# bdwsq1996/Effi-MVS-plus

Hardware: AMD Instinct MI355X
Metric: ref-views/sec (cost-volume hot path: warp + cost volume + 3-D regularisation + cascaded GRU refinement) (higher is better)
Workload: dtype f32 (3x3 MFMA convs: products as 3 bf16 partial products hi*hi+hi*lo+lo*hi, f32 accumulate; all else f32); 1 GPU; cfg3: DTU-shaped 1600x1184, N=5 views (S=4 sources), 3-stage cascade ndepths=48,8,8, GRU iters 3,3,3, seeded-random weights, features of the stock FPN resident in HBM; parallelism=single GPU, views_in_flight=3, arithmetic=split

## Files before the change

effi_mvs_plus_amd/_lib.py:

```python
from __future__ import annotations

import ctypes as C
import os
import threading

_HERE = os.path.dirname(os.path.abspath(__file__))
LIB_PATH = os.environ.get("EFFI_MVS_LIB") or os.path.join(_HERE, "libeffimvs_hip.so")
HEADER_PATH = os.path.join(os.path.dirname(_HERE), "include", "effi_mvs_hip.h")

_vp, _i, _l, _f, _d = C.c_void_p, C.c_int, C.c_long, C.c_float, C.c_double

SIGNATURES = {
    "effi_version": [],
    "effi_set_workspace": [_i, _vp, _l],
    "effi_set_option": [C.c_char_p, _l],
    "effi_launch_form": [_i, _i, _i, _i, _i, _i, _i, _i, _vp],
    "effi_fusion_dynamic_filter_f32": [_vp, _vp, _vp, _vp, _i, _i, _i, _vp, _i, _i, _f, _i, _f, _f, _i, _vp, _vp, _vp, _vp, _vp, _vp,
                                       _vp, _vp],
    "effi_fusion_dtu_filter_f32": [_vp, _vp, _vp, _vp, _i, _i, _i, _vp, _f, _f, _i, _i, _f, _f, _vp, _vp, _vp, _vp, _vp, _vp, _vp],
    "effi_fusion_dtu_filter_scan_f32": [_vp, _vp, _i, _vp, _vp, _i, _i, _i, _i, _vp, _f, _f, _i, _i, _f, _f, _vp, _vp, _vp, _vp, _vp, _vp, _vp],
    "effi_fusion_dynamic_filter_scan_f32": [_vp, _vp, _i, _vp, _vp, _i, _i, _i, _i, _vp, _i, _i, _f, _i, _f, _f, _i, _vp, _vp, _vp, _vp, _vp,
                                            _vp, _vp],
    "effi_fusion_static_filter_f32": [_vp, _vp, _vp, _vp, _i, _i, _i, _vp, _i, _i, _f, _d, _d, _d, _vp, _vp, _vp, _vp, _vp, _vp, _vp, _vp,
                                      _vp],
# ... 10 lines not shown
    "effi_fusion_gipuma_view_f32": [_vp, _vp, _vp, _i, _i, _vp, _vp, _i, _i, _i, _f, _i, _f, _f, _vp, _vp, _vp, _vp, _vp, _vp, _vp],
    "effi_dtu_cell_keys_f32": [_vp, _l, _d, _i, _i, _i, _i, _i, _i, _vp, _vp],
    "effi_dtu_reduce_blocks": [_l],
    "effi_dtu_reduce_round_f32": [_vp, _vp, _l, _i, _i, _i, _d, _vp, _vp, _vp, _vp],
    "effi_dtu_nn_capped_f32": [_vp, _l, _vp, _vp, _l, _d, _i, _i, _i, _i, _i, _i, _d, _vp, _vp],
    "effi_dtu_obs_mask_f32": [_vp, _l, _d, _d, _d, _d, _vp, _i, _i, _i, _vp, _vp],
    "effi_dtu_above_plane_f32": [_vp, _l, _d, _d, _d, _d, _vp, _vp],
    "effi_metrics_blocks": [_l],
    "effi_mvs_loss_f32": [_vp, _vp, _vp, _vp, _i, _i, _vp, _vp, _vp, _vp, _vp, _vp],
    "effi_mvs_loss_bwd_f32": [_vp, _vp, _vp, _vp, _i, _i, _vp, _vp, _vp, _vp, _vp],
    "effi_depth_metrics_f32": [_vp, _vp, _vp, _i, _l, _i, _vp, _i, _vp, _vp, _i, _vp, _vp, _vp, _vp, _vp, _vp],
    "effi_adamw_max_tensors": [],
    "effi_adamw_multi_f32": [_vp, _vp, _vp, _vp, _vp, _vp, _i, _d, _vp, _d, _d, _d, _d, _vp],
    "effi_gradnorm_max_tensors": [],
    "effi_gradnorm_chunks": [_vp, _i],
    "effi_gradnorm_partial_f32": [_vp, _vp, _i, _vp, _vp],
    "effi_gradnorm_finish_f32": [_vp, _l, _d, _vp, _vp, _vp],
    "effi_adamw_multi_clip_f32": [_vp, _vp, _vp, _vp, _vp, _vp, _i, _d, _vp, _d, _d, _d, _d, _vp, _i, _vp],
    "effi_fusion_vis_filter_f32": [_vp, _vp, _i, _i, _i, _i, _f, _f, _i, _i, _vp, _vp],
    "effi_fusion_points_f32": [_i, _vp, _l, _vp, _vp, _i, _i, _i, _vp, _vp, _vp],
    "effi_fusion_dtu_reproject_f32": [_vp, _vp, _vp, _vp, _i, _i, _i, _i, _f, _f, _vp, _vp, _vp, _vp],
    "effi_compose_rel_proj_f32": [_vp, _i, _vp, _vp],
    "effi_rel_proj_f32": [_vp, _vp, _vp, _vp],
    "effi_planar_to_nhwc_f32": [_vp, _vp, _i, _i, _i, _vp],
    "effi_homo_warp_f32": [_vp, _vp, _vp, _l, _l, _i, _i, _i, _i, _vp, _vp],
    "effi_warpcorr_views_f32": [_vp, _vp, _i, _vp, _vp, _l, _l, _i, _i, _i, _i, _vp, _vp, _vp],
    "effi_warpcorr_views_tbl_f32": [_vp, _i, _vp, _vp, _l, _l, _i, _i, _i, _i, _vp, _vp, _vp],
    "effi_warpcorr_views_x3_f32": [_vp, _vp, _i, _vp, _vp, _l, _l, _i, _i, _i, _i, _vp, _vp, _i, _vp],
    "effi_warpcorr_views_x3_tbl_f32": [_vp, _i, _vp, _vp, _l, _l, _i, _i, _i, _i, _vp, _vp, _i, _vp],
    "effi_warpcorr_dyn_tbl_f32": [_vp, _i, _vp, _vp, _vp, _vp, _i, _i, _i, _i, _i, _vp, _vp, _vp],
    "effi_view_table_set": [_vp, _vp, _i, _vp],
    "effi_pixelwise_net_f32": [_vp, _vp, _i, _i, _i, _vp, _vp],
    "effi_view_aggregate_f32": [_vp, _vp, _i, _i, _i, _vp, _vp],
    "effi_warpcorr_dyn_f32": [_vp, _vp, _i, _vp, _vp, _vp, _vp, _i, _i, _i, _i, _i, _vp, _vp, _vp],
    "effi_conv3d_k3_f32": [_vp, _vp, _i, _vp, _vp, _i, _i, _i, _i, _i, _i, _i, _vp, _vp, _vp],
    "effi_deconv3d_k3s2_bf16x3_f32": [_vp, _i, _vp, _vp, _i, _i, _i, _i, _i, _vp, _vp, _vp],
    "effi_conv3d_k3s2_mfma_f32": [_vp, _i, _vp, _vp, _i, _i, _i, _i, _i, _vp, _vp],
    "effi_conv3d_k3s1_mfma_f32": [_vp, _i, _vp, _vp, _i, _i, _i, _i, _i, _vp, _vp],
    "effi_deconv3d_k3_f32": [_vp, _i, _vp, _vp, _i, _i, _i, _i, _i, _i, _vp, _vp, _vp],
    "effi_softmax_regress_conf_f32": [_vp, _vp, _l, _l, _i, _i, _vp, _vp, _vp, _i, _vp, _vp],
    "effi_softmax_regress_conf_up_f32": [_vp, _vp, _l, _l, _i, _i, _i, _vp, _vp, _vp, _i, _vp, _vp, _i, _vp],
    "effi_vol_lookup1d_f32": [_vp, _l, _l, _i, _vp, _l, _l, _l, _i, _vp, _vp, _l, _i, _i, _vp, _vp],
    "effi_bilinear_sampler1d_f32": [_vp, _i, _i, _i, _vp, _l, _vp, _vp, _vp],
    "effi_getcost_conv1x1_f32": [_vp, _vp, _i, _i, _vp, _vp, _l, _l, _i, _vp, _l, _l, _i, _vp, _vp, _l, _i, _i, _i, _vp, _vp, _i,
                                 _i, _vp, _vp],
    "effi_getcost_f32": [_vp, _vp, _i, _i, _vp, _vp, _l, _l, _i, _vp, _l, _l, _i, _vp, _vp, _l, _i, _i, _i, _vp, _vp],
    "effi_conv2d_f32": [_vp, _vp, _i, _vp, _vp, _i, _i, _i, _i, _i, _i, _vp, _vp, _vp, _i, _vp, _vp, _vp],
    "effi_conv3d_k3s1_roll_bf16x3_f32": [_vp, _vp, _i, _vp, _vp, _i, _i, _i, _i, _i, _vp, _vp],
    "effi_conv3d_k3s1_bf16x3_f32": [_vp, _vp, _i, _vp, _vp, _i, _i, _i, _i, _i, _vp, _vp],
    "effi_vol_lookup1d_pair_f32": [_vp, _vp, _l, _l, _i, _vp, _l, _l, _l, _i, _vp, _vp, _l, _i, _i, _vp, _vp, _vp],
    "effi_conv3d_k3_pair_f32": [_vp, _vp, _vp, _vp, _vp, _vp, _vp, _vp, _i, _i, _i, _i, _i, _i, _i, _vp],
    "effi_conv3d_k3s1_roll_bf16x3_pair_f32": [_vp, _vp, _vp, _vp, _vp, _vp, _vp, _vp, _vp, _i, _i, _i, _i, _i, _i, _vp],
    "effi_csp_gen_roll_bf16x3_pair_f32": [_vp, _i, _i, _i] + [_vp] * 16 + [_vp],
    "effi_debug_poison_lds": [C.c_uint, _vp, _vp],
    "effi_debug_pk_war_probe": [_vp, _i, _i, _i, _vp],
    "effi_deconv3d_k3_pair_f32": [_vp, _vp, _vp, _vp, _vp, _vp, _vp, _vp, _i, _i, _i, _i, _i, _i, _i, _vp],
    "effi_homo_warp_bwd_f32": [_vp, _vp, _l, _l, _i, _i, _i, _i, _vp, _vp, _vp],
    "effi_warpcorr_views_bwd_f32": [_vp, _vp, _i, _vp, _vp, _l, _l, _i, _i, _i, _i, _vp, _vp, _vp, _vp],
    "effi_image_prepare_u8_f32": [_vp, _i, _i, _i, _i, _i, _vp, _vp],
    "effi_resize_linear_f32": [_vp, _i, _i, _i, _i, _i, _vp, _vp],
    "effi_images_prepare_batch_u8_f32": [_vp, _i, _i, _i, _vp, _vp],
    "effi_gt_pyramid_f32": [_vp, _vp, _i, _vp, _i, _i, _i, _vp, _vp, _vp],
    "effi_encoder_inputs_f32": [_vp, _vp, _i, _vp, _vp, _l, _l, _i, _vp, _l, _l, _i, _vp, _vp, _l, _i, _i, _i, _vp, _vp, _vp, _vp,
                                _i, _vp, _vp, _vp],
    "effi_encoder_inputs_bf16x3_f32": [_vp, _vp, _i, _vp, _vp, _l, _l, _i, _vp, _l, _l, _i, _vp, _vp, _l, _i, _i, _i, _vp, _vp, _vp, _vp,
                                       _i, _vp, _vp, _vp],
    "effi_conv2d_k3_bf16x3_pair_f32": [_vp, _vp, _i, _vp, _vp, _vp, _vp, _vp, _i, _vp, _vp, _vp, _i, _i, _i, _i, _vp],
    "effi_conv2d_k3_k1_up2x_bf16x3_f32": [_vp, _vp, _i, _vp, _vp, _i, _vp, _vp, _vp, _vp, _i, _i, _i, _vp, _vp, _vp],
    "effi_conv2d_k3_k1_bf16x3_f32": [_vp, _vp, _i, _vp, _vp, _i, _i, _vp, _i, _vp, _vp, _i, _i, _i, _i, _vp, _vp],
    "effi_conv2d_k3_bf16x3_f32": [_vp, _vp, _i, _vp, _vp, _i, _i, _i, _i, _i, _vp, _vp, _vp, _i, _vp, _vp, _vp],
    "effi_conv2d_k5s2_f32": [_vp, _i, _vp, _vp, _i, _i, _i, _i, _vp, _vp],
    "effi_conv2d_k5s2_bf16x3_f32": [_vp, _i, _vp, _vp, _i, _i, _i, _i, _vp, _vp],
    "effi_conv3d_k3s2_bf16x3_f32": [_vp, _i, _vp, _vp, _i, _i, _i, _i, _i, _vp, _vp],
    "effi_conv2d_c1k7_relu_f32": [_vp, _vp, _vp, _i, _i, _i, _vp, _vp],
    "effi_conv2d_c1k7_relu_bf16x3_f32": [_vp, _vp, _vp, _i, _i, _i, _vp, _vp],
    "effi_convex_upsample2x_f32": [_vp, _vp, _vp, _i, _i, _i, _vp, _vp, _vp, _vp],
    "effi_compose_rel_proj_stages_f32": [_vp, _i, _i, _vp, _vp],
    "effi_cascade_setup_f32": [_vp, _i, _i, _vp, _vp, _vp, _i, _i, _vp, _vp],
    "effi_split_tanh_relu_stages_f32": [_vp, _vp, _vp, _vp, _vp, _vp, _i, _vp],
    "effi_split_tanh_relu_f32": [_vp, _i, _i, _i, _vp, _vp, _vp],
    "effi_depth_to_inv_f32": [_vp, _vp, _i, _i, _vp, _vp],
    "effi_stage1_hypotheses_f32": [_vp, _i, _i, _vp, _vp, _vp],
    "effi_upsample_nearest_f32": [_vp, _i, _i, _i, _i, _vp, _vp],
    "effi_head_update_f32": [_vp, _vp, _vp, _vp, _i, _i, _i, _vp, _vp, _vp],
    "effi_conv2d_k3_twice_bf16x3_f32": [_vp, _i, _vp, _vp, _vp, _vp, _i, _i, _i, _vp, _vp],
    "effi_conv2d_f32_batch": [_vp, _vp, _i, _vp, _vp, _i, _i, _i, _i, _i, _i, _vp, _vp, _vp, _i, _vp, _vp, _i, _vp, _l, _l, _vp],
    "effi_conv2d_k3_bf16x3_f32_batch": [_vp, _vp, _i, _vp, _vp, _i, _i, _i, _i, _i, _vp, _vp, _vp, _i, _vp, _vp, _i, _vp, _l, _l, _vp],
    "effi_conv2d_k5s2_f32_batch": [_vp, _i, _vp, _vp, _i, _i, _i, _i, _vp, _i, _l, _l, _vp],
    "effi_conv2d_k5s2_bf16x3_f32_batch": [_vp, _i, _vp, _vp, _i, _i, _i, _i, _vp, _i, _l, _l, _vp],
    "effi_conv2d_k3_twice_bf16x3_f32_batch": [_vp, _i, _vp, _vp, _vp, _vp, _i, _i, _i, _vp, _i, _l, _l, _vp],
    "effi_compose_rel_proj_f32_batch": [_vp, _i, _vp, _i, _l, _l, _vp],
    "effi_cascade_setup_f32_batch": [_vp, _i, _i, _vp, _vp, _vp, _i, _i, _vp, _i, _l, _l, _l, _vp, _l, _vp],
    "effi_warpcorr_views_f32_batch": [_vp, _vp, _i, _vp, _vp, _l, _l, _i, _i, _i, _i, _vp, _vp, _i, _l, _l, _l, _l, _l, _l, _vp],
    "effi_warpcorr_views_x3_f32_batch": [_vp, _vp, _i, _vp, _vp, _l, _l, _i, _i, _i, _i, _vp, _vp, _i, _i, _l, _l, _l, _l, _l, _l, _vp],
    "effi_view_aggregate_f32_batch": [_vp, _vp, _i, _i, _i, _vp, _i, _l, _l, _l, _vp],
    "effi_softmax_regress_conf_f32_batch": [_vp, _vp, _l, _l, _i, _i, _vp, _vp, _vp, _i, _vp, _i, _l, _l, _l, _l, _l, _l, _vp],
    "effi_softmax_regress_conf_up_f32_batch": [_vp, _vp, _l, _l, _i, _i, _i, _vp, _vp, _vp, _i, _vp, _vp, _i, _i, _l, _l, _l, _l, _l, _l,
                                               _l, _vp],
    "effi_conv3d_k3_f32_batch": [_vp, _vp, _i, _vp, _vp, _i, _i, _i, _i, _i, _i, _i, _vp, _vp, _i, _vp, _l, _l, _vp],
    "effi_deconv3d_k3_f32_batch": [_vp, _i, _vp, _vp, _i, _i, _i, _i, _i, _i, _vp, _vp, _i, _l, _l, _l, _vp],
    "effi_conv3d_k3s1_mfma_f32_batch": [_vp, _i, _vp, _vp, _i, _i, _i, _i, _i, _vp, _i, _l, _l, _vp],
    "effi_conv3d_k3s2_mfma_f32_batch": [_vp, _i, _vp, _vp, _i, _i, _i, _i, _i, _vp, _i, _l, _l, _vp],
    "effi_conv3d_k3s1_bf16x3_f32_batch": [_vp, _vp, _i, _vp, _vp, _i, _i, _i, _i, _i, _vp, _i, _vp, _l, _vp],
    "effi_conv3d_k3s1_roll_bf16x3_f32_batch": [_vp, _vp, _i, _vp, _vp, _i, _i, _i, _i, _i, _vp, _i, _vp, _l, _vp],
    "effi_conv3d_k3s2_bf16x3_f32_batch": [_vp, _i, _vp, _vp, _i, _i, _i, _i, _i, _vp, _i, _l, _l, _vp],
    "effi_deconv3d_k3s2_bf16x3_f32_batch": [_vp, _i, _vp, _vp, _i, _i, _i, _i, _i, _vp, _vp, _i, _l, _l, _l, _vp],
# ... 106 lines not shown
```

effi_mvs_plus_amd/csrc/api.hip:

```cpp
#include "common.hpp"
#include "launch_form.hpp"
#include <cstdlib>
#include <cstring>
#include <mutex>

extern "C" int effi_version(void) { return 200; }

extern "C" const char* effi_error_string(int code) {
    switch (code) {
        case EFFI_OK: return "ok";
        case EFFI_ERR_BADARG: return "bad argument (null pointer, non-positive size, or inconsistent shapes)";
        case EFFI_ERR_UNSUPPORTED: return "shape / channel count not instantiated in this build";
        case EFFI_ERR_LAUNCH: return "kernel launch failed (hipPeekAtLastError)";
        case EFFI_ERR_WORKSPACE: return "no workspace registered for the current device (effi_set_workspace)";
        default: return "unknown error code";
    }
}

static const void* g_workspace[EFFI_MAX_DEVICES];

extern "C" long effi_workspace_bytes(void) { return 256; }

extern "C" int effi_set_workspace(int device, void* workspace, long bytes) {
    if (device < 0 || device >= EFFI_MAX_DEVICES) return EFFI_ERR_BADARG;
    if (workspace != nullptr && bytes < effi_workspace_bytes()) return EFFI_ERR_BADARG;
    __atomic_store_n(&g_workspace[device], (const void*)workspace, __ATOMIC_RELEASE);
    return EFFI_OK;
}

extern "C" const void* effi_get_workspace(int device) {
    if (device < 0 || device >= EFFI_MAX_DEVICES) return nullptr;
    return __atomic_load_n(&g_workspace[device], __ATOMIC_ACQUIRE);
}

const float* effi_zero_page() {
    int dev = -1;
    if (hipGetDevice(&dev) != hipSuccess) return nullptr;
    return (const float*)effi_get_workspace(dev);
}

namespace {
const char* const kOptName[EFFI_OPT_COUNT] = {"warp_lds_kb", "dyn_form", "dyn_setup_exact", "dyn_xchg", "pixnet_mfma", "force_mr", "mr4_min",
                                              "mr4_nt2_max", "mr2_min", "wide_tiles", "roll_mr", "roll_zt", "roll_rp", "deconv_mr", "sr_waves", "enc_gen_mr3", "c3_lean", "dyn_win",
                                              "roll_slide"};
long g_opt[EFFI_OPT_COUNT];
std::once_flag g_opt_once;
void load_options() {
    for (int i = 0; i < EFFI_OPT_COUNT; ++i) {
        char env[64] = "EFFI_";
        size_t n = strlen(env);
        for (const char* c = kOptName[i]; *c && n + 1 < sizeof(env); ++c) env[n++] = (*c >= 'a' && *c <= 'z') ? (char)(*c - 32) : *c;
        env[n] = 0;
        const char* v = getenv(env);
        g_opt[i] = (v && *v) ? atol(v) : EFFI_OPT_UNSET;
    }
}
int find_option(const char* name) {
    if (!name) return -1;
    for (int i = 0; i < EFFI_OPT_COUNT; ++i)
        if (strcmp(name, kOptName[i]) == 0) return i;
    return -1;
}
}

long effi_option(int id) {
    std::call_once(g_opt_once, load_options);
    return __atomic_load_n(&g_opt[id], __ATOMIC_RELAXED);
}

extern "C" int effi_set_option(const char* name, long value) {
    const int id = find_option(name);
    if (id < 0) return EFFI_ERR_BADARG;
    std::call_once(g_opt_once, load_options);
    __atomic_store_n(&g_opt[id], value, __ATOMIC_RELAXED);
    return EFFI_OK;
}

extern "C" long effi_get_option(const char* name) {
    const int id = find_option(name);
    return id < 0 ? EFFI_OPT_UNSET : effi_option(id);
}

extern "C" long effi_option_unset(void) { return EFFI_OPT_UNSET; }

extern "C" int effi_launch_form(int launcher, int nt, int h, int w, int planes, int count, int cout, int flags, int* form) {
    if (!form || nt < 1 || h < 1 || w < 1 || planes < 1 || count < 1 || cout < 1) return EFFI_ERR_BADARG;
    const bool sr = flags & EFFI_LF_FLAG_SR, zb = flags & EFFI_LF_FLAG_ZB, k1 = flags & EFFI_LF_FLAG_K1, s2 = flags & EFFI_LF_FLAG_S2;
    const EffiFormOpts o = effi_form_opts();
    EffiForm f;
    switch (launcher) {
        case EFFI_LF_X3: f = effi_pick_x3(nt, h, w, zb ? planes : 1, zb, sr, o); break;
        case EFFI_LF_X3_BATCH: f = effi_pick_x3_batch(nt, h, w, count, o); break;
        case EFFI_LF_X3_ZB_BATCH: f = effi_pick_x3_zb_batch(nt, h, w, (long)planes * count, o); break;
        case EFFI_LF_X3_PAIR: f = effi_pick_x3_pair(nt, h, w, sr, o); break;
        case EFFI_LF_CONV2D: f = effi_pick_generic(k1 ? 1 : 3, h, w, count); break;
        case EFFI_LF_PLANES3D: f = effi_pick_planes(h, w, (long)planes * count, s2 ? 2 : 4); break;
        case EFFI_LF_K5S2: f = effi_pick_planes(h, w, count, 2); break;
        case EFFI_LF_S2_X3: f = effi_pick_s2_x3(h, w, nt == 1 ? 1 : (nt + 1) / 2, (long)planes * count); break;
        case EFFI_LF_ROLL: f = effi_pick_roll((flags & EFFI_LF_FLAG_OCT2) ? 2 : 1, nt, cout, h, w, planes, count, o); break;
        case EFFI_LF_DECONV_X3: f = effi_pick_deconv_x3(cout, h, w, planes, count, o); break;
        case EFFI_LF_C3_PLANES: f = effi_pick_c3_planes(h, w, planes, count); break;
        case EFFI_LF_DECONV_K3: f = effi_pick_deconv_k3(cout, h, w, planes, count); break;
        case EFFI_LF_C3_ZPT: f = EffiForm{1, EFFI_C3_TX, 4, effi_pick_c3_zpt(s2 ? 2 : 1, s2 ? 2 : 1, h, w, planes, nt, count), 0}; break;
        default: return EFFI_ERR_BADARG;
    }
    form[0] = f.rows, form[1] = f.cols, form[2] = f.waves, form[3] = f.planes, form[4] = f.variant;
    return EFFI_OK;
}

namespace {
__global__ __launch_bounds__(256) void lds_poison_kernel(unsigned pattern, unsigned* sink) {
    __shared__ unsigned buf[16 * 1024];
    for (int i = threadIdx.x; i < 16 * 1024; i += 256) buf[i] = pattern;
    __syncthreads();
    if (buf[(threadIdx.x * 61) & 16383] != pattern) sink[0] = 1;
}
}

extern "C" int effi_debug_poison_lds(unsigned pattern, void* sink4, effi_stream_t stream) {
    if (!sink4) return EFFI_ERR_BADARG;
    hipLaunchKernelGGL(lds_poison_kernel, dim3(2048), dim3(256), 0, effi_s(stream), pattern, reinterpret_cast<unsigned*>(sink4));
    EFFI_LAUNCH_CHECK();
    return EFFI_OK;
}

namespace {
template <int VARIANT>
__global__ __launch_bounds__(256) void pk_war_probe_kernel(float* __restrict__ out, int reps) {
    const int tid = blockIdx.x * 256 + threadIdx.x;
    const float x = 1.0f + (float)(tid & 15) * 0.0625f, y = 2.0f, bad = 1000.0f, w = 1.0f;
    float r0, r1;
    asm volatile(
        "v_mov_b32 v10, %2\n"
        "v_mov_b32 v11, %3\n"
        "v_mov_b32 v12, 0\n"
        "v_mov_b32 v13, 0\n"
        "v_mov_b32 v14, %5\n"
        "v_mov_b32 v15, %5\n"
        "s_nop 7\n"
        "s_mov_b32 s20, %6\n"
        "1:\n"
        ".rept 16\n"
        ".if %c7 == 3\n"
        "v_fma_f32 v12, v10, v14, v12\n"
        "v_fma_f32 v13, v11, v14, v13\n"
        ".else\n"
        "v_pk_fma_f32 v[12:13], v[10:11], v[14:15], v[12:13] op_sel_hi:[1,0,1]\n"
        ".endif\n"
        ".if %c7 == 1\n"
        "s_nop 0\n"
        ".endif\n"
        ".if %c7 == 2\n"
        "v_pk_mov_b32 v[10:11], v[16:17], v[10:11] op_sel:[0,1]\n"
        ".else\n"
// ... 31 lines not shown
```

effi_mvs_plus_amd/csrc/common.hpp:

```cpp
#pragma once
#include <hip/hip_runtime.h>
#include "../../include/effi_mvs_hip.h"

#define EFFI_LAUNCH_CHECK()                                   \
    do {                                                      \
        if (hipPeekAtLastError() != hipSuccess) return EFFI_ERR_LAUNCH; \
    } while (0)

const float* effi_zero_page();

enum EffiOption {
    EFFI_OPT_WARP_LDS_KB,
    EFFI_OPT_DYN_FORM,
    EFFI_OPT_DYN_SETUP_EXACT,
    EFFI_OPT_DYN_XCHG,
    EFFI_OPT_PIXNET_MFMA,
    EFFI_OPT_FORCE_MR,
    EFFI_OPT_MR4_MIN, EFFI_OPT_MR4_NT2_MAX, EFFI_OPT_MR2_MIN,
    EFFI_OPT_WIDE_TILES,
    EFFI_OPT_ROLL_MR, EFFI_OPT_ROLL_ZT, EFFI_OPT_ROLL_RP,
    EFFI_OPT_DECONV_MR,
    EFFI_OPT_SR_WAVES,
    EFFI_OPT_ENC_GEN_MR3,
    EFFI_OPT_C3_LEAN,
    EFFI_OPT_DYN_WIN,
    EFFI_OPT_ROLL_SLIDE,
    EFFI_OPT_COUNT
};
constexpr long EFFI_OPT_UNSET = -0x7fffffffL;
long effi_option(int id);

static inline hipStream_t effi_s(effi_stream_t s) {
    (void)hipGetLastError();
    return reinterpret_cast<hipStream_t>(s);
}
static inline int effi_cdiv(long a, long b) { return (int)((a + b - 1) / b); }

struct EffiPtrList {
    const float* p[EFFI_MAX_VIEWS + 1];
    const float* const* tbl;
};
__device__ __forceinline__ const float* effi_resolve_views(const float* ref, const EffiPtrList& l) {
    return l.tbl ? l.tbl[0] : ref;
}
struct EffiOutList {
    float* p[EFFI_MAX_VIEWS + 1];
};

__device__ __forceinline__ float effi_dpp_f(float v, int ctrl_sel) {
    int i = __float_as_int(v);
    int r;
    switch (ctrl_sel) {
        case 0:  r = __builtin_amdgcn_update_dpp(0, i, 0xB1, 0xF, 0xF, true); break;
        case 1:  r = __builtin_amdgcn_update_dpp(0, i, 0x4E, 0xF, 0xF, true); break;
        default: r = __builtin_amdgcn_update_dpp(0, i, 0x141, 0xF, 0xF, true); break;
    }
    return __int_as_float(r);
}

template <int LPP>
__device__ __forceinline__ float effi_group_sum(float v) {
    static_assert(LPP == 1 || LPP == 2 || LPP == 4 || LPP == 8, "lanes per pixel");
    if (LPP >= 2) v += effi_dpp_f(v, 0);
    if (LPP >= 4) v += effi_dpp_f(v, 1);
    if (LPP >= 8) v += effi_dpp_f(v, 2);
    return v;
}
template <int LPP>
__device__ __forceinline__ float effi_group_max(float v) {
    if (LPP >= 2) v = fmaxf(v, effi_dpp_f(v, 0));
    if (LPP >= 4) v = fmaxf(v, effi_dpp_f(v, 1));
    if (LPP >= 8) v = fmaxf(v, effi_dpp_f(v, 2));
    return v;
}

__device__ __forceinline__ int effi_xcd_remap(int bid, int nblocks) {
    const int q = nblocks >> 3, r = nblocks & 7;
    const int xcd = bid & 7, idx = bid >> 3;
    const int base = (xcd < r) ? xcd * (q + 1) : r * (q + 1) + (xcd - r) * q;
// ... 54 lines not shown
        intervals[threadIdx.x] = base * ratio;
    } else if (threadIdx.x == 3) {
        intervals[3] = 1.0f / hi;
    } else if (threadIdx.x == 4) {
        intervals[4] = 1.0f / lo;
    }
}

__device__ __forceinline__ float effi_lk_rcp(float b) {
#ifdef EFFI_EXACT_LOOKUP
    return 1.0f / b;
#else
    const float r0 = __builtin_amdgcn_rcpf(b);
    return fmaf(fmaf(-b, r0, 1.0f), r0, r0);
#endif
}
__device__ __forceinline__ float effi_lk_div(float a, float b, float rb) {
#ifdef EFFI_EXACT_LOOKUP
    (void)rb;
    return a / b;
#else
    const float q = a * rb;
    return fmaf(fmaf(-q, b, a), rb, q);
#endif
}

__device__ __forceinline__ void lookup1d_index(int Dp, float q_depth, float dmin, float dmax, int& x0, float& w0, float& w1) {
    const float scaled = effi_lk_rcp(q_depth);
    const float min_disp = effi_lk_rcp(dmax), max_disp = effi_lk_rcp(dmin);
    const float den = (max_disp - min_disp) + 1e-10f;
    const float disp = effi_lk_div(scaled - min_disp, den, effi_lk_rcp(den));
    const float dm1 = (float)(Dp - 1);
    const float t = disp * dm1;
    const float g = effi_lk_div(2.0f * t, dm1, effi_lk_rcp(dm1)) - 1.0f;
    float ix = ((g + 1.0f) * 0.5f) * dm1;
    ix = fminf(fmaxf(ix, -2.0f), dm1 + 2.0f);
    const float x0f = floorf(ix);
    x0 = (int)x0f;
    w1 = ix - x0f;
    w0 = (x0f + 1.0f) - ix;
}
__device__ __forceinline__ int lookup1d_tap0(int Dp, int x0) { return min(max(x0, 0), Dp - 1); }
__device__ __forceinline__ int lookup1d_tap1(int Dp, int x0) { return min(max(x0 + 1, 0), Dp - 1); }
__device__ __forceinline__ float lookup1d_blend(int Dp, int x0, float w0, float w1, float v0, float v1) {
    const bool in0 = (x0 >= 0) & (x0 <= Dp - 1), in1 = (x0 + 1 >= 0) & (x0 + 1 <= Dp - 1);
    float r = in0 ? v0 * w0 : 0.0f;
    r = in1 ? r + v1 * w1 : r;
    return r;
}
__device__ __forceinline__ float lookup1d_fetch(const float* __restrict__ vol, long dstride, int Dp, int x0, float w0, float w1) {
    const float v0 = vol[lookup1d_tap0(Dp, x0) * dstride], v1 = vol[lookup1d_tap1(Dp, x0) * dstride];
    return lookup1d_blend(Dp, x0, w0, w1, v0, v1);
}
__host__ __device__ inline bool effi_vol_fits32(long npix, long ps, int D, long ds) {
    return ps >= 0 && ds >= 0 && npix >= 1 && D >= 1 && ((npix - 1) * ps + (long)(D - 1) * ds + 1) * 4 < (1L << 31);
}
__host__ __device__ inline bool effi_lookup_fits32(long npix, long cps, int Dcur, long cds, long rps, int Dreg, long rds) {
    return effi_vol_fits32(npix, cps, Dcur, cds) && effi_vol_fits32(npix, rps, Dreg, rds);
}
template <int NQ>
__device__ __forceinline__ void effi_getcost_pixel(float inv_or_depth, int input_is_depth, const float* __restrict__ disp_range, int n_range,
                                                   float itv, const float* __restrict__ cur_vol, long cpo, long cds, int Dcur,
                                                   const float* __restrict__ reg_vol, long rpo, long rds, int Dreg, float rlo, float rhi,
                                                   bool off32, float (&cost)[2 * NQ]) {
    float depth = inv_or_depth;
    if (!input_is_depth) depth = effi_inv_to_depth(depth, disp_range[0], disp_range[n_range - 1]);
    const float dv = effi_lk_rcp(depth);
    const float half = (float)(NQ / 2) * itv;
    const float smin = fmaxf(dv - half, 1e-4f);
    const float smax = fminf(fmaxf(dv + half, 1e-4f), 1e4f);
    const float step = (smax - smin) / (float)(NQ - 1);
    constexpr int QB = NQ <= 3 ? NQ : 2;
    static_assert(NQ % QB == 0, "whole batches");
#pragma unroll
    for (int k0 = 0; k0 < NQ; k0 += QB) {
        int xc[QB], xr[QB];
        float wc0[QB], wc1[QB], wr0[QB], wr1[QB];
#pragma unroll
        for (int k = 0; k < QB; ++k) {
            const float s = fmaxf(smin + (float)(k0 + k) * step, 1e-5f);
            const float qd = effi_lk_rcp(s);
            lookup1d_index(Dcur, qd, rlo, rhi, xc[k], wc0[k], wc1[k]);
            xr[k] = xc[k]; wr0[k] = wc0[k]; wr1[k] = wc1[k];
            if (Dreg != Dcur) lookup1d_index(Dreg, qd, rlo, rhi, xr[k], wr0[k], wr1[k]);
        }
        float vc0[QB], vc1[QB], vr0[QB], vr1[QB];
        if (off32) {
            const unsigned cb = (unsigned)cpo * 4u, rb = (unsigned)rpo * 4u, cs = (unsigned)cds * 4u, rs = (unsigned)rds * 4u;
            const char* cbase = reinterpret_cast<const char*>(cur_vol);
            const char* rbase = reinterpret_cast<const char*>(reg_vol);
#pragma unroll
            for (int k = 0; k < QB; ++k) {
                vc0[k] = *reinterpret_cast<const float*>(cbase + (size_t)(cb + (unsigned)lookup1d_tap0(Dcur, xc[k]) * cs));
                vc1[k] = *reinterpret_cast<const float*>(cbase + (size_t)(cb + (unsigned)lookup1d_tap1(Dcur, xc[k]) * cs));
                vr0[k] = *reinterpret_cast<const float*>(rbase + (size_t)(rb + (unsigned)lookup1d_tap0(Dreg, xr[k]) * rs));
                vr1[k] = *reinterpret_cast<const float*>(rbase + (size_t)(rb + (unsigned)lookup1d_tap1(Dreg, xr[k]) * rs));
            }
        } else {
            const float* __restrict__ cur = cur_vol + cpo;
            const float* __restrict__ reg = reg_vol + rpo;
#pragma unroll
            for (int k = 0; k < QB; ++k) {
                vc0[k] = cur[lookup1d_tap0(Dcur, xc[k]) * cds];
                vc1[k] = cur[lookup1d_tap1(Dcur, xc[k]) * cds];
                vr0[k] = reg[lookup1d_tap0(Dreg, xr[k]) * rds];
                vr1[k] = reg[lookup1d_tap1(Dreg, xr[k]) * rds];
// ... 192 lines not shown
```

effi_mvs_plus_amd/csrc/conv3d.hip:

```cpp
#include "common.hpp"
#include "launch_form.hpp"

namespace {

constexpr int TX = EFFI_C3_TX, TY = EFFI_C3_TY;
static_assert(TX * TY == 256, "one thread per tile pixel");

struct SrcSet {
    const float* p[EFFI_MAX_SRC];
    int ch[EFFI_MAX_SRC];
};

__device__ __forceinline__ const float* src_channel(const SrcSet& s, int c, long plane) {
    if (c < s.ch[0]) return s.p[0] + (long)c * plane;
    c -= s.ch[0];
    if (c < s.ch[1]) return s.p[1] + (long)c * plane;
    c -= s.ch[1];
    return s.p[2] + (long)c * plane;
}

template <int COUT_T, int SZ, int SXY, int ZPT, bool DENSE>
__device__ __forceinline__ void conv3d_k3_body(SrcSet src, int cin, const float* __restrict__ wgt,
                                               const float* __restrict__ bias, int cout,
                                               int D, int h, int w, int Do, int ho, int wo,
// ... 121 lines not shown

template <int COUT_T, int SZ, int SXY, int ZPT, bool DENSE = false>
__global__ __launch_bounds__(256) void conv3d_k3_kernel(SrcSet src, int cin, const float* __restrict__ wgt,
                                                        const float* __restrict__ bias, int cout,
                                                        int D, int h, int w, int Do, int ho, int wo,
                                                        int relu, const float* __restrict__ skip,
                                                        float* __restrict__ out) {
    conv3d_k3_body<COUT_T, SZ, SXY, ZPT, DENSE>(src, cin, wgt, bias, cout, D, h, w, Do, ho, wo, relu, skip, out);
}

struct C3Batch {
    long src[EFFI_MAX_SRC];
    long skip, out;
};
template <int COUT_T, int SZ, int SXY, int ZPT, bool DENSE = false>
__global__ __launch_bounds__(256) void conv3d_k3_batch_kernel(SrcSet src, C3Batch bt, int cin, const float* __restrict__ wgt,
                                                              const float* __restrict__ bias, int cout, int D, int h, int w, int Do,
                                                              int ho, int wo, int relu, const float* __restrict__ skip,
                                                              float* __restrict__ out) {
    const long smp = blockIdx.y;
#pragma unroll
    for (int i = 0; i < EFFI_MAX_SRC; ++i) src.p[i] += smp * bt.src[i];
    conv3d_k3_body<COUT_T, SZ, SXY, ZPT, DENSE>(src, cin, wgt, bias, cout, D, h, w, Do, ho, wo, relu, skip ? skip + smp * bt.skip : nullptr,
                                                out + smp * bt.out);
}

struct Conv3dCall {
    SrcSet src;
    const float* wgt;
    const float* bias;
    const float* skip;
    float* out;
};
template <int COUT_T, int SZ, int SXY, int ZPT>
__global__ __launch_bounds__(256) void conv3d_k3_pair_kernel(Conv3dCall a, Conv3dCall b, int cin, int cout, int D, int h, int w,
                                                             int Do, int ho, int wo, int relu) {
    const bool second = blockIdx.y != 0;
    SrcSet src;
#pragma unroll
    for (int i = 0; i < EFFI_MAX_SRC; ++i) {
        src.p[i] = second ? b.src.p[i] : a.src.p[i];
        src.ch[i] = second ? b.src.ch[i] : a.src.ch[i];
    }
    conv3d_k3_body<COUT_T, SZ, SXY, ZPT, true>(src, cin, second ? b.wgt : a.wgt, second ? b.bias : a.bias, cout, D, h, w, Do, ho, wo,
                                               relu, second ? b.skip : a.skip, second ? b.out : a.out);
}

struct C1Call {
    const float* in;
    const float* wgt;
    const float* bias;
    float* out;
};
template <int SXY, int ZPT>
__device__ __forceinline__ void conv3d_c1to8_body(const float* __restrict__ in, const float* __restrict__ wgt, const float* __restrict__ bias,
                                                  float* __restrict__ out, int D, int h, int w, int ho, int wo, int relu) {
    constexpr int IZ = ZPT + 2, IY = (TY - 1) * SXY + 3, IX = (TX - 1) * SXY + 3;
    constexpr int PSZ = IY * IX, NPL = (PSZ + 255) / 256, PSZP = NPL * 256;
    __shared__ float tile[IZ * PSZP];
    __shared__ __attribute__((aligned(16))) float wl[27 * 8 + 8];

    const int tid = threadIdx.x;
    const int tiles_x = (wo + TX - 1) / TX, tiles_xy = tiles_x * ((ho + TY - 1) / TY);
    int lid = effi_xcd_remap(blockIdx.x, gridDim.x);
    const int tile_xy = lid % tiles_xy, zg = lid / tiles_xy;
    const int by = tile_xy / tiles_x, bx = tile_xy - by * tiles_x;
    const int tx = tid % TX, ty = tid / TX;
    const int ox = bx * TX + tx, oy = by * TY + ty, oz0 = zg * ZPT;
    const int iz0 = oz0 - 1, iy0 = by * TY * SXY - 1, ix0 = bx * TX * SXY - 1;

    if (tid < 27 * 8) wl[tid] = wgt[tid];
    if (tid < 8) wl[27 * 8 + tid] = bias ? bias[tid] : 0.0f;

    int poff[NPL];
#pragma unroll
    for (int k = 0; k < NPL; ++k) {
        const int e = tid + k * 256;
        const int ly = e / IX, lx = e - ly * IX;
        const int gy = iy0 + ly, gx = ix0 + lx;
        poff[k] = ((e < PSZ) & (gy >= 0) & (gy < h) & (gx >= 0) & (gx < w)) ? gy * w + gx : -1;
    }
    float pf[IZ][NPL];
    unsigned pb[NPL];
#pragma unroll
    for (int k = 0; k < NPL; ++k) pb[k] = (unsigned)max(poff[k], 0) * 4u;
    const unsigned plane_b = (unsigned)(h * w) * 4u;
#pragma unroll
    for (int lz = 0; lz < IZ; ++lz) {
        const int gz = iz0 + lz;
        const bool zok = (gz >= 0) & (gz < D);
        const unsigned so = (unsigned)min(max(gz, 0), D - 1) * plane_b;
#pragma unroll
        for (int k = 0; k < NPL; ++k) {
            const float t = *reinterpret_cast<const float*>(reinterpret_cast<const char*>(in) + (so + pb[k]));
            pf[lz][k] = (zok & (poff[k] >= 0)) ? t : 0.0f;
        }
    }
#pragma unroll
    for (int lz = 0; lz < IZ; ++lz)
#pragma unroll
        for (int k = 0; k < NPL; ++k) tile[lz * PSZP + tid + k * 256] = pf[lz][k];
    __syncthreads();

    typedef float f2 __attribute__((ext_vector_type(2)));
    typedef float f4 __attribute__((ext_vector_type(4)));
    f2 acc[ZPT][4];
#pragma unroll
    for (int z = 0; z < ZPT; ++z)
#pragma unroll
        for (int c = 0; c < 4; ++c) acc[z][c] = f2{0.0f, 0.0f};
    const float* tc = tile + (ty * SXY) * IX + tx * SXY;
#pragma unroll 1
    for (int t = 0; t < 9; ++t) {
        const int ky = t / 3, kx = t - 3 * ky;
        float col[IZ];
#pragma unroll
        for (int z = 0; z < IZ; ++z) col[z] = tc[z * PSZP + ky * IX + kx];
#pragma unroll
        for (int kd = 0; kd < 3; ++kd) {
            const f4 w0 = *reinterpret_cast<const f4*>(&wl[(kd * 9 + t) * 8]);
            const f4 w1 = *reinterpret_cast<const f4*>(&wl[(kd * 9 + t) * 8 + 4]);
            const f2 wk[4] = {f2{w0[0], w0[1]}, f2{w0[2], w0[3]}, f2{w1[0], w1[1]}, f2{w1[2], w1[3]}};
#pragma unroll
            for (int z = 0; z < ZPT; ++z) {
                const f2 cv = {col[z + kd], col[z + kd]};
#pragma unroll
                for (int c = 0; c < 4; ++c) acc[z][c] = __builtin_elementwise_fma(cv, wk[c], acc[z][c]);
            }
        }
    }

    if (ox >= wo || oy >= ho) return;
    const long out_plane = (long)D * ho * wo;
    float bv[8];
#pragma unroll
    for (int co = 0; co < 8; ++co) bv[co] = wl[27 * 8 + co];
#pragma unroll
    for (int z = 0; z < ZPT; ++z) {
        const int oz = oz0 + z;
        if (oz >= D) break;
        const long o = ((long)oz * ho + oy) * wo + ox;
#pragma unroll
        for (int co = 0; co < 8; ++co) {
            float v = acc[z][co >> 1][co & 1] + bv[co];
            if (relu) v = fmaxf(v, 0.0f);
            out[(long)co * out_plane + o] = v;
        }
    }
}

template <int SXY, int ZPT>
__global__ __launch_bounds__(256) void conv3d_c1to8_kernel(C1Call ca, C1Call cb, int D, int h, int w, int ho, int wo, int relu) {
    const bool second = blockIdx.y != 0;
    conv3d_c1to8_body<SXY, ZPT>(second ? cb.in : ca.in, second ? cb.wgt : ca.wgt, second ? cb.bias : ca.bias, second ? cb.out : ca.out, D, h,
                                w, ho, wo, relu);
}
template <int SXY, int ZPT>
__global__ __launch_bounds__(256) void conv3d_c1to8_batch_kernel(C1Call c, long in_ss, long out_ss, int D, int h, int w, int ho, int wo,
                                                                 int relu) {
    const long smp = blockIdx.y;
    conv3d_c1to8_body<SXY, ZPT>(c.in + smp * in_ss, c.wgt, c.bias, c.out + smp * out_ss, D, h, w, ho, wo, relu);
}

static bool c3_lean(int bit) {
    const long v = effi_option(EFFI_OPT_C3_LEAN);
    return v == EFFI_OPT_UNSET || ((v >> bit) & 1);
}

static bool route_c1to8(int cin, int cout, int sz, int sxy, const float* skip) {
    return cin == 1 && cout == 8 && sz == 1 && (sxy == 1 || sxy == 2) && !skip && c3_lean(0);
}
static bool route_c8to1(int cin, int cout, int sz, const float* skip) { return cin == 8 && cout == 1 && sz == 1 && !skip && c3_lean(1); }

struct C3Samples {
    int n;
    C3Batch ss;
};

int launch_c1to8(const C1Call& a, const C1Call* b, int D, int h, int w, int sxy, int relu, hipStream_t st, const C3Samples* bt = nullptr) {
    if (!effi_c1to8_fits32(D, h, w)) return EFFI_ERR_UNSUPPORTED;
    const int ho = (h - 1) / sxy + 1, wo = (w - 1) / sxy + 1, ncall = b ? 2 : bt ? bt->n : 1;
    const int planes = effi_pick_c3_planes(ho, wo, D, ncall).planes;
    const dim3 grid(effi_cdiv(wo, TX) * effi_cdiv(ho, TY) * effi_cdiv(D, planes), ncall);
    return effi_switch<1, 2>(sxy, [&](auto SXY) {
        return effi_switch<4, 8>(planes, [&](auto ZPT) {
            if (bt) return effi_launch<conv3d_c1to8_batch_kernel<SXY(), ZPT()>>(grid, 256, st, a, bt->ss.src[0], bt->ss.out, D, h, w, ho, wo, relu);
            return effi_launch<conv3d_c1to8_kernel<SXY(), ZPT()>>(grid, 256, st, a, b ? *b : a, D, h, w, ho, wo, relu);
        });
    });
}

struct C8Call {
    const float* in;
    const float* wgt;
    const float* bias;
    float* out;
};
template <bool DECONV, int ZPT>
__device__ __forceinline__ void conv3d_c8to1_body(const float* __restrict__ in, const float* __restrict__ wgt, const float* __restrict__ bias,
                                                  float* __restrict__ out, int D, int h, int w, int relu) {
#ifndef EFFI_C8_CC
#define EFFI_C8_CC 2
#endif
    constexpr int IZ = ZPT + 2, CC = (ZPT == 8) ? 1 : EFFI_C8_CC;
    constexpr int IY = DECONV ? TY + 1 : TY + 2, IX = DECONV ? TX + 1 : TX + 2;
#ifndef EFFI_C8_PADMASK
#define EFFI_C8_PADMASK 127
#endif
    constexpr int PSZ = IY * IX, PSZP = (PSZ + EFFI_C8_PADMASK) & ~EFFI_C8_PADMASK, NPL = (PSZP + 255) / 256, LASTN = PSZP - 256 * (NPL - 1);
    __shared__ float tile[CC * IZ * PSZP];
    __shared__ __attribute__((aligned(16))) float wl[8 * 28 + 4];

    const int tid = threadIdx.x;
    const int tiles_x = (w + TX - 1) / TX, tiles_xy = tiles_x * ((h + TY - 1) / TY);
    int lid = effi_xcd_remap(blockIdx.x, gridDim.x);
    const int tile_xy = lid % tiles_xy, zg = lid / tiles_xy;
    const int by = tile_xy / tiles_x, bx = tile_xy - by * tiles_x;
    const int tx = tid % TX, ty = tid / TX;
    const int ix = bx * TX + tx, iy = by * TY + ty, z0 = zg * ZPT;
    const int iz0 = z0 - 1, iy0 = DECONV ? by * TY : by * TY - 1, ix0 = DECONV ? bx * TX : bx * TX - 1;
    const long in_plane = (long)D * h * w;

    if (tid < 8 * 27) wl[(tid / 27) * 28 + tid % 27] = wgt[tid];
    if (tid < 8) wl[tid * 28 + 27] = 0.0f;
    if (tid == 0) wl[8 * 28] = bias ? bias[0] : 0.0f;

    int poff[NPL];
#pragma unroll
    for (int k = 0; k < NPL; ++k) {
        const int e = tid + k * 256;
        const int ly = e / IX, lx = e - ly * IX;
        const int gy = iy0 + ly, gx = ix0 + lx;
        poff[k] = ((e < PSZ) & (gy >= 0) & (gy < h) & (gx >= 0) & (gx < w)) ? gy * w + gx : -1;
    }
    const bool last_pass = tid < LASTN;

    typedef float f4 __attribute__((ext_vector_type(4)));
    constexpr int NACC = DECONV ? ZPT * 4 : ZPT;
    float acc[NACC];
#pragma unroll
    for (int i = 0; i < NACC; ++i) acc[i] = 0.0f;
// ... 86 lines not shown
                                        const int kd = az + 2 - lz;
                                        if (kd < 0 || kd > 2) continue;
                                        acc[(az * 2 + ay) * 2 + ax] = fmaf(v, wk[kd * 9 + ky * 3 + kx], acc[(az * 2 + ay) * 2 + ax]);
                                    }
                                }
                            }
                        }
            }
        }
    }

    if (ix >= w || iy >= h) return;
    const float b = wl[8 * 28];
    if constexpr (!DECONV) {
#pragma unroll
        for (int z = 0; z < ZPT; ++z) {
            const int oz = z0 + z;
            if (oz >= D) break;
            float v = acc[z] + b;
            if (relu) v = fmaxf(v, 0.0f);
            out[((long)oz * h + iy) * w + ix] = v;
        }
    } else {
        const int ho = 2 * h, wo = 2 * w;
#pragma unroll
        for (int az = 0; az < ZPT; ++az) {
            const int oz = z0 + az;
            if (oz >= D) break;
#pragma unroll
            for (int ay = 0; ay < 2; ++ay) {
                float v0 = acc[(az * 2 + ay) * 2] + b, v1 = acc[(az * 2 + ay) * 2 + 1] + b;
                if (relu) { v0 = fmaxf(v0, 0.0f); v1 = fmaxf(v1, 0.0f); }
                *reinterpret_cast<float2*>(out + ((long)oz * ho + 2 * iy + ay) * wo + 2 * ix) = make_float2(v0, v1);
            }
        }
    }
}

template <bool DECONV, int ZPT>
__global__ __launch_bounds__(256) void conv3d_c8to1_kernel(C8Call ca, C8Call cb, int D, int h, int w, int relu) {
    const bool second = blockIdx.y != 0;
    conv3d_c8to1_body<DECONV, ZPT>(second ? cb.in : ca.in, second ? cb.wgt : ca.wgt, second ? cb.bias : ca.bias, second ? cb.out : ca.out, D,
                                   h, w, relu);
}
template <bool DECONV, int ZPT>
__global__ __launch_bounds__(256) void conv3d_c8to1_batch_kernel(C8Call c, long in_ss, long out_ss, int D, int h, int w, int relu) {
    const long smp = blockIdx.y;
    conv3d_c8to1_body<DECONV, ZPT>(c.in + smp * in_ss, c.wgt, c.bias, c.out + smp * out_ss, D, h, w, relu);
}

template <bool DECONV>
int launch_c8to1(const C8Call& a, const C8Call* b, int D, int h, int w, int relu, hipStream_t st, const C3Samples* bt = nullptr) {
    if (!effi_c8to1_fits32(D, h, w)) return EFFI_ERR_UNSUPPORTED;
    const int ncall = b ? 2 : bt ? bt->n : 1, planes = effi_pick_c3_planes(h, w, D, ncall).planes;
    const dim3 grid(effi_cdiv(w, TX) * effi_cdiv(h, TY) * effi_cdiv(D, planes), ncall);
    return effi_switch<4, 8>(planes, [&](auto ZPT) {
        if (bt) return effi_launch<conv3d_c8to1_batch_kernel<DECONV, ZPT()>>(grid, 256, st, a, bt->ss.src[0], bt->ss.out, D, h, w, relu);
        return effi_launch<conv3d_c8to1_kernel<DECONV, ZPT()>>(grid, 256, st, a, b ? *b : a, D, h, w, relu);
    });
}

template <int COUT_T, int SZ>
__device__ __forceinline__ void deconv3d_k3_body(const float* __restrict__ in, int cin,
                                                 const float* __restrict__ wgt,
                                                 const float* __restrict__ bias, int cout,
                                                 int D, int h, int w, int relu,
                                                 const float* __restrict__ skip, float* __restrict__ out) {
    constexpr int ZPT = (SZ == 2) ? 1 : 4;
    constexpr int OZ = (SZ == 2) ? 2 : ZPT;
    constexpr int CC = 4;
    constexpr int IZ = (SZ == 2) ? 2 : ZPT + 2, IY = TY + 1, IX = TX + 1;
    constexpr int PLANE = IZ * IY * IX;
    constexpr int PSZ = IY * IX, NPL = (PSZ + 255) / 256;
    __shared__ float tile[CC * PLANE];

    const int tiles_x = (w + TX - 1) / TX, tiles_xy = tiles_x * ((h + TY - 1) / TY), nzg = (D + ZPT - 1) / ZPT;
    int lid = effi_xcd_remap(blockIdx.x, gridDim.x);
    const int tile_xy = lid % tiles_xy;
    lid /= tiles_xy;
    const int zg = lid % nzg, cg = lid / nzg;
    const int by = tile_xy / tiles_x, bx = tile_xy - by * tiles_x;
    const int tx = threadIdx.x % TX, ty = threadIdx.x / TX;
    const int ix = bx * TX + tx, iy = by * TY + ty, z0 = zg * ZPT;
    const int co0 = cg * COUT_T;
    const int iz0 = (SZ == 2) ? z0 : z0 - 1;
    const long in_plane = (long)D * h * w;

    int poff[NPL];
#pragma unroll
    for (int k = 0; k < NPL; ++k) {
        const int e = threadIdx.x + k * 256;
        const int ly = e / IX, lx = e - ly * IX;
        const int gy = by * TY + ly, gx = bx * TX + lx;
        poff[k] = ((e < PSZ) & (gy < h) & (gx < w)) ? gy * w + gx : -1;
    }

    float acc[OZ][2][2][COUT_T];
#pragma unroll
    for (int a = 0; a < OZ; ++a)
#pragma unroll
        for (int b = 0; b < 2; ++b)
#pragma unroll
            for (int c = 0; c < 2; ++c)
#pragma unroll
                for (int d = 0; d < COUT_T; ++d) acc[a][b][c][d] = 0.0f;

    float pf[CC][IZ][NPL];
// ... 264 lines not shown

extern "C" int effi_conv3d_k3_f32_batch(const float* const* srcs, const int* src_channels, int n_src, const float* weight,
                                        const float* bias, int cout, int D, int h, int w, int sz, int sxy, int relu,
                                        const float* skip, float* out, int n_smp, const long* src_sstride, long skip_sstride,
                                        long out_sstride, effi_stream_t stream) {
    C3Samples b;
    if (const int rc = fill_samples(b, n_smp, src_sstride, n_src, skip_sstride, out_sstride)) return rc;
    return conv3d_k3_impl(srcs, src_channels, n_src, weight, bias, cout, D, h, w, sz, sxy, relu, skip, out, n_smp > 1 ? &b : nullptr, stream);
}

static int deconv3d_k3_impl(const float* in, int cin, const float* weight, const float* bias, int cout, int D, int h, int w, int sz,
                            int relu, const float* skip, float* out, const C3Samples* bt, effi_stream_t stream) {
    Deconv3dCall c;
    if (cout < 1) return EFFI_ERR_BADARG;
    if (const int rc = fill_deconv(c, in, weight, bias, skip, out, cin, D, h, w)) return rc;
    return deconv3d_k3_run(c, nullptr, cin, cout, D, h, w, sz, relu, bt, stream);
}

extern "C" int effi_deconv3d_k3_f32(const float* in, int cin, const float* weight, const float* bias, int cout, int D,
                                    int h, int w, int sz, int relu, const float* skip, float* out,
                                    effi_stream_t stream) {
    return deconv3d_k3_impl(in, cin, weight, bias, cout, D, h, w, sz, relu, skip, out, nullptr, stream);
}

extern "C" int effi_deconv3d_k3_f32_batch(const float* in, int cin, const float* weight, const float* bias, int cout, int D, int h,
                                          int w, int sz, int relu, const float* skip, float* out, int n_smp, long in_sstride,
                                          long skip_sstride, long out_sstride, effi_stream_t stream) {
    C3Samples b;
    if (const int rc = fill_samples(b, n_smp, &in_sstride, 1, skip_sstride, out_sstride)) return rc;
    return deconv3d_k3_impl(in, cin, weight, bias, cout, D, h, w, sz, relu, skip, out, n_smp > 1 ? &b : nullptr, stream);
}

extern "C" int effi_conv3d_k3_pair_f32(const float* in_a, const float* weight_a, const float* bias_a, float* out_a,
                                       const float* in_b, const float* weight_b, const float* bias_b, float* out_b, int cin,
                                       int cout, int D, int h, int w, int sxy, int relu, effi_stream_t stream) {
    Conv3dCall a, b;
    int cin_a, cin_b;
    if (fill_conv(a, cin_a, &in_a, &cin, 1, weight_a, bias_a, nullptr, out_a, D, h, w) ||
        fill_conv(b, cin_b, &in_b, &cin, 1, weight_b, bias_b, nullptr, out_b, D, h, w))
        return EFFI_ERR_BADARG;
    if (cout != 8 || (sxy != 1 && sxy != 2)) return EFFI_ERR_UNSUPPORTED;
    return conv3d_k3_run(a, &b, cin, cout, D, h, w, 1, sxy, relu, nullptr, stream);
}

extern "C" int effi_deconv3d_k3_pair_f32(const float* in_a, const float* weight_a, const float* bias_a, float* out_a,
                                         const float* in_b, const float* weight_b, const float* bias_b, float* out_b, int cin,
                                         int cout, int D, int h, int w, int sz, int relu, effi_stream_t stream) {
    Deconv3dCall a, b;
    if (fill_deconv(a, in_a, weight_a, bias_a, nullptr, out_a, cin, D, h, w) || fill_deconv(b, in_b, weight_b, bias_b, nullptr, out_b, cin, D, h, w))
        return EFFI_ERR_BADARG;
    if (sz != 1 || cout != 1) return EFFI_ERR_UNSUPPORTED;
    return deconv3d_k3_run(a, &b, cin, cout, D, h, w, sz, relu, nullptr, stream);
}
```

effi_mvs_plus_amd/csrc/launch_form.hpp:

```cpp
#pragma once
#include "common.hpp"
#include <type_traits>

template <int... Vs, class F>
static int effi_switch_or(int miss, long v, F&& f) {
    int rc = miss;
    (void)(... || (v == Vs ? (rc = f(std::integral_constant<int, Vs>{}), true) : false));
    return rc;
}
template <int... Vs, class F>
static int effi_switch(long v, F&& f) { return effi_switch_or<Vs...>(EFFI_ERR_BADARG, v, f); }
template <int... Vs, class F>
static int effi_switch_nt(long v, F&& f) { return effi_switch_or<Vs...>(EFFI_ERR_UNSUPPORTED, v, f); }

template <auto KERNEL, class... Args>
static int effi_launch_lds(dim3 grid, int threads, size_t dynamic_lds, hipStream_t st, const Args&... args) {
    hipLaunchKernelGGL(KERNEL, grid, dim3(threads), dynamic_lds, st, args...);
    return hipPeekAtLastError() == hipSuccess ? EFFI_OK : EFFI_ERR_LAUNCH;
}
template <auto KERNEL, class... Args>
static int effi_launch(dim3 grid, int threads, hipStream_t st, const Args&... args) {
    return effi_launch_lds<KERNEL>(grid, threads, 0, st, args...);
}

#ifndef EFFI_C3_TX
#define EFFI_C3_TX 32
#define EFFI_C3_TY 8
#endif

struct EffiFormOpts {
    long force_mr;
    long mr4_min, mr4_nt2_max, mr2_min;
    long wide_tiles;
    long sr_waves, roll_mr, roll_zt, roll_rp, deconv_mr;
    long roll_slide;
};

static inline long effi_opt_or(int id, long dflt) {
    const long v = effi_option(id);
    return v == EFFI_OPT_UNSET ? dflt : v;
}

static inline EffiFormOpts effi_form_opts() {
    EffiFormOpts o;
    o.force_mr = effi_opt_or(EFFI_OPT_FORCE_MR, 0);
    o.mr4_min = effi_opt_or(EFFI_OPT_MR4_MIN, 400);
    o.mr4_nt2_max = effi_opt_or(EFFI_OPT_MR4_NT2_MAX, 1024);
    o.mr2_min = effi_opt_or(EFFI_OPT_MR2_MIN, 400);
    o.wide_tiles = effi_opt_or(EFFI_OPT_WIDE_TILES, -1);
    o.sr_waves = effi_option(EFFI_OPT_SR_WAVES);
    o.roll_mr = effi_option(EFFI_OPT_ROLL_MR);
    o.roll_zt = effi_option(EFFI_OPT_ROLL_ZT);
    o.roll_rp = effi_option(EFFI_OPT_ROLL_RP);
    o.deconv_mr = effi_option(EFFI_OPT_DECONV_MR);
    o.roll_slide = effi_opt_or(EFFI_OPT_ROLL_SLIDE, 1);
    return o;
}

struct EffiForm {
    int rows;
    int cols;
    int waves;
    int planes;
    int variant;
};

static inline int effi_pick_x3_rows(int nt, int h, int w, long count, const EffiFormOpts& o) {
    const long cols = effi_cdiv(w, 16);
    const long t4 = cols * effi_cdiv(h, 16) * count, t2 = cols * effi_cdiv(h, 8) * count;
    int mr;
    if (t4 >= o.mr4_min && !(nt == 2 && t4 >= o.mr4_nt2_max)) mr = 4;
    else if (t2 >= o.mr2_min) mr = 2;
    else mr = 1;
    if (o.force_mr) mr = (int)o.force_mr;
    return mr;
}

static inline EffiForm effi_pick_x3(int nt, int h, int w, long planes, bool zb, bool sr, const EffiFormOpts& o) {
    const int mr = effi_pick_x3_rows(nt, h, w, planes, o);
    const bool wide = o.wide_tiles >= 0 ? o.wide_tiles != 0 : (mr == 4 && w >= 512 && !zb);
    if (wide) return EffiForm{mr, 16 * mr, 4, 1, 1};
    if (sr && ((o.sr_waves == 8 && mr <= 2) || (o.sr_waves == EFFI_OPT_UNSET && mr == 1 && nt >= 6))) return EffiForm{mr, 16, 8, 1, 0};
    return EffiForm{mr, 16, 4, 1, 0};
}

static inline EffiForm effi_pick_x3_batch(int nt, int h, int w, long n_img, const EffiFormOpts& o) {
    const int mr = effi_pick_x3_rows(nt, h, w, n_img, o);
    const bool wide = o.wide_tiles >= 0 ? o.wide_tiles != 0 : (mr == 4 && w >= 512);
    return wide ? EffiForm{mr, 16 * mr, 4, 1, 1} : EffiForm{mr, 16, 4, 1, 0};
}

static inline EffiForm effi_pick_x3_zb_batch(int nt, int h, int w, long planes, const EffiFormOpts& o) {
    return EffiForm{effi_pick_x3_rows(nt, h, w, planes, o), 16, 4, 1, 0};
}

static inline EffiForm effi_pick_x3_pair(int nt, int h, int w, bool sr, const EffiFormOpts& o) {
    const int mr = effi_pick_x3_rows(nt, h, w, 2, o);
    if (mr == 4 && w >= 512) return EffiForm{4, 64, 4, 1, 1};
    if (sr && o.sr_waves == 8 && mr <= 2) return EffiForm{mr, 16, 8, 1, 0};
    return EffiForm{mr, 16, 4, 1, 0};
}

static inline EffiForm effi_pick_generic(int ks, int h, int w, long n_img) {
    if (w & 3) return EffiForm{0, 16, 4, 1, 0};
    const long cols = effi_cdiv(w, 16);
    const long t4 = cols * effi_cdiv(h, 16) * n_img, t2 = cols * effi_cdiv(h, 8) * n_img;
    int mr;
    if (t4 >= 512 || (ks == 1 && t4 >= 256)) mr = 4;
    else if (t2 >= 512 || ks == 1) mr = 2;
    else mr = 1;
    return EffiForm{mr, 16, 4, 1, 0};
}

static inline EffiForm effi_pick_planes(int h, int w, long planes, int max_rows) {
    const long cols = effi_cdiv(w, 16);
    if (max_rows >= 4 && cols * effi_cdiv(h, 16) * planes >= 512) return EffiForm{4, 16, 4, 1, 0};
    if (cols * effi_cdiv(h, 8) * planes >= 512) return EffiForm{2, 16, 4, 1, 0};
    return EffiForm{1, 16, 4, 1, 0};
}

static inline EffiForm effi_pick_s2_x3(int h, int w, int ngroups, long planes) {
    const int cols = effi_cdiv(w, 16);
    return EffiForm{(long)cols * effi_cdiv(h, 8) * ngroups * planes >= 400 ? 2 : 1, 16, 4, 1, 0};
}

static inline EffiForm effi_pick_roll(int noct, int nt, int cout, int h, int w, int D, long mult, const EffiFormOpts& o) {
    const int cols = effi_cdiv(w, 16);
    const bool rp = nt == 1 && cout <= 8 && o.roll_rp != 0;
    int mr = 2, zt = D;
    double best = 1e30;
    for (int m = 2; m <= 4; m += 2) {
        const int occ = rp ? (noct == 1 ? 3 : 2) : (noct == 1 && nt == 1) ? (m == 2 ? 3 : 2) : (noct == 1 ? 2 : (nt == 1 && m == 2 ? 2 : 1));
        const long tiles_m = (long)cols * effi_cdiv(h, 4 * m), slots = 256L * occ;
        for (int nz = 1; nz <= D; ++nz) {
            const int z = effi_cdiv(D, nz);
            const long wgs = tiles_m * effi_cdiv(D, z) * mult;
            const double cost = (double)effi_cdiv(wgs, slots) * (z + 3) * (m == 4 ? 1.3 : 1.0);
            if (cost < best - 1e-9) { best = cost; mr = m; zt = z; }
        }
    }
    if (o.roll_mr != EFFI_OPT_UNSET) mr = (int)o.roll_mr;
    if (o.roll_zt != EFFI_OPT_UNSET) zt = (int)o.roll_zt;
    return EffiForm{mr, 16, 4, zt, rp ? 1 : 0};
}

static inline EffiForm effi_pick_deconv_x3(int cout, int h, int w, int D, long n_smp, const EffiFormOpts& o) {
    const int tiles_x = effi_cdiv(w, 16);
    const bool al = (w & 3) == 0, half = cout <= 8;
    const int occ1 = half ? ((n_smp > 1 && !al) ? 4 : 5) : 3, occ2 = half ? 3 : 2;
    const long wg1 = (long)tiles_x * effi_cdiv(h, 4) * D * n_smp, wg2 = (long)tiles_x * effi_cdiv(h, 8) * D * n_smp;
    bool mr2 = effi_cdiv(wg2, 256L * occ2) * 4 < effi_cdiv(wg1, 256L * occ1) * 3;
    if (o.deconv_mr != EFFI_OPT_UNSET) mr2 = o.deconv_mr == 2;
    return EffiForm{mr2 ? 2 : 1, 16, 4, 1, 0};
}

static inline EffiForm effi_pick_c3_planes(int h, int w, int D, long ncall) {
    const long tiles = (long)effi_cdiv(w, EFFI_C3_TX) * effi_cdiv(h, EFFI_C3_TY);
    return EffiForm{1, EFFI_C3_TX, 4, tiles * effi_cdiv(D, 8) * ncall >= 512 ? 8 : 4, 0};
}

static inline bool effi_c1to8_fits32(int D, int h, int w) { return (long)D * h * w < (1L << 29); }
static inline bool effi_c8to1_fits32(int D, int h, int w) { return 8L * D * h * w < (1L << 29); }

constexpr int effi_c3_zbig(int sz, int sxy) { return (sxy == 1 || sz == 1) ? 4 : 2; }
static inline int effi_pick_c3_zpt(int sz, int sxy, int ho, int wo, int Do, int cout_tiles, long ncall) {
    const int zbig = effi_c3_zbig(sz, sxy);
    const long blocks = (long)effi_cdiv(wo, EFFI_C3_TX) * effi_cdiv(ho, EFFI_C3_TY) * effi_cdiv(Do, zbig) * cout_tiles * ncall;
    return blocks >= 384 ? zbig : 1;
}
constexpr int EFFI_LF_C3_ZPT = 12;

static inline EffiForm effi_pick_deconv_k3(int cout, int h, int w, int D, long n_smp) {
    const int tiles = effi_cdiv(w, EFFI_C3_TX) * effi_cdiv(h, EFFI_C3_TY);
    return EffiForm{1, EFFI_C3_TX, 4, (long)tiles * D * (cout / 8) * n_smp >= 512 ? 8 : 4, 0};
}

struct EffiWarpOpts {
    long warp_lds_kb, dyn_form, dyn_setup_exact, dyn_win;
};
static inline EffiWarpOpts effi_warp_opts() {
    return EffiWarpOpts{effi_option(EFFI_OPT_WARP_LDS_KB), effi_option(EFFI_OPT_DYN_FORM), effi_option(EFFI_OPT_DYN_SETUP_EXACT),
                        effi_option(EFFI_OPT_DYN_WIN)};
}

constexpr int EFFI_WIN_MAXPX = 576;

static inline int effi_warp_lds_px(const EffiWarpOpts& o) {
    if (o.warp_lds_kb == EFFI_OPT_UNSET) return EFFI_WIN_MAXPX;
    if (o.warp_lds_kb < 0) return -1;
    const long px = o.warp_lds_kb * 1024 / 128;
    return px < EFFI_WIN_MAXPX ? (int)px : EFFI_WIN_MAXPX;
}

enum EffiViewsKernel { EFFI_VIEWS_GATHER, EFFI_VIEWS_WINDOW, EFFI_VIEWS_MM };
struct EffiViewsForm {
    EffiViewsKernel kernel;
    int lds_px;
};
static inline EffiViewsForm effi_pick_views(bool x3, int C, long dps, int D, int h, int w, const EffiWarpOpts& o) {
    const bool shared = C == 32 && dps == 0 && D <= 256;
    if (x3 && shared && h < 32000 && w < 32000) return EffiViewsForm{EFFI_VIEWS_MM, 0};
    const int lds_px = effi_warp_lds_px(o);
    if (shared && lds_px >= 0) return EffiViewsForm{EFFI_VIEWS_WINDOW, lds_px};
    return EffiViewsForm{EFFI_VIEWS_GATHER, 0};
}

enum EffiDynKernel { EFFI_DYN_EXACT, EFFI_DYN_SPLIT, EFFI_DYN_HYP, EFFI_DYN_WINDOW };
struct EffiDynForm {
    EffiDynKernel kernel;
    int lds_px;
};
// ... 7 lines not shown
```

effi_mvs_plus_amd/csrc/vol_host_check.cpp:

```cpp
#include "host_check_record.hpp"
#include "conv3d.hip"
#include "volume_ops.hip"

static void show_one(const EffiPtrList& l) {
    for (int i = 0; i <= EFFI_MAX_VIEWS; ++i) ptr(L("p%d", i).c_str(), l.p[i]);
    FP(l, tbl);
}
static void show_one(const EffiOutList& l) {
    for (int i = 0; i <= EFFI_MAX_VIEWS; ++i) ptr(L("p%d", i).c_str(), l.p[i]);
}
#define FA(s, f, n) do { for (int i_ = 0; i_ < (n); ++i_) if ((s).f[i_] != 0) put(" " #f "%d=%ld", i_, (long)(s).f[i_]); } while (0)
#define FPA(s, f, n) do { for (int i_ = 0; i_ < (n); ++i_) ptr(L(#f "%d", i_).c_str(), (s).f[i_]); } while (0)
namespace {
void show_one(const SrcSet& s) { FPA(s, p, EFFI_MAX_SRC); FA(s, ch, EFFI_MAX_SRC); }
void show_one(const C3Batch& b) { FA(b, src, EFFI_MAX_SRC); FI(b, skip), FI(b, out); }
void show_one(const Conv3dCall& c) { show_one(c.src); FP(c, wgt), FP(c, bias), FP(c, skip), FP(c, out); }
void show_one(const C1Call& c) { FP(c, in), FP(c, wgt), FP(c, bias), FP(c, out); }
void show_one(const C8Call& c) { FP(c, in), FP(c, wgt), FP(c, bias), FP(c, out); }
void show_one(const Deconv3dCall& c) { FP(c, in), FP(c, wgt), FP(c, bias), FP(c, skip), FP(c, out); }
void show_one(const SoftmaxBatch& b) {
    FI(b, logits), FI(b, depth), FI(b, out_depth), FI(b, out_conf), FI(b, range), FI(b, out_dinv), FI(b, out_conf_up);
}
void show_one(const GetcostConvArgs& g) {
    FP(g, inv_depth), FP(g, disp_range), FI(g, n_range), FI(g, input_is_depth), FP(g, interval);
    FP(g, cur_vol), FI(g, cds), FI(g, cps), FI(g, Dcur), FP(g, reg_vol), FI(g, rds), FI(g, rps), FI(g, Dreg);
    FP(g, dmin), FP(g, dmax), FI(g, range_ps), FI(g, hw), FP(g, weight), FP(g, bias), FI(g, cout), FI(g, relu), FP(g, out);
    FP(g, out_sr), FP(g, out7_sr), FI(g, w), FI(g, sr_hp), FI(g, sr_wp), FI(g, off32);
}
void show_one(const SplitStages& a) {
    FPA(a, ctx, 4); FPA(a, hidden, 4); FPA(a, inp, 4); FA(a, nh, 4); FA(a, n, 4); FA(a, first, 5); FI(a, vec4);
}
void show_one(const SrMaps& a) { FPA(a, base, 4); FA(a, planes, 4); FA(a, h, 4); FA(a, w, 4); FA(a, hp, 4); FA(a, wp, 4); FA(a, first, 5); }
void show_one(const SplitStagesSr& a) {
    FPA(a, ctx, 4); FPA(a, hidden, 4); FPA(a, inp, 4); FPA(a, hidden_sr, 4);
    FA(a, hd, 4); FA(a, cd, 4); FA(a, h, 4); FA(a, w, 4); FA(a, hp, 4); FA(a, wp, 4); FA(a, q4, 4); FA(a, first, 5);
    FPA(a, clear_base, 4); FA(a, clear_planes, 4); FA(a, nsplit, 4);
}
}

static void direct_failure(const std::string& what) {
    std::printf("FAILED: %s\n", what.c_str());
    ++g_failures;
}
template <class T> static T* off(T* p, long floats) { return reinterpret_cast<T*>(reinterpret_cast<uintptr_t>(p) + 4 * floats); }

static const float* const SRCS[4] = {P(2), P(3), P(4), P(5)};
static const float* const SRCS_NULL1[3] = {P(2), nullptr, P(4)};
struct ConvArgs {
    const float* const* srcs = SRCS;
    int ch[4] = {8, 4, 3, 2};
    bool null_ch = false, null_ss = false;
    int n_src = 1;
    const float* wgt = P(10);
    const float* bias = P(11);
    int cout = 8, D = 6, h = 37, w = 50, sz = 1, sxy = 1, relu = 1;
    const float* skip = nullptr;
    float* out = P(13);
    int n_smp = 3;
    long ss[3] = {1000, 2000, 3000}, skip_ss = 4000, out_ss = 5000;
};
static std::string conv(bool batch, const std::string& label, const ConvArgs& a) {
    g_rec.clear();
    const int rc = batch ? effi_conv3d_k3_f32_batch(a.srcs, (a.null_ch ? nullptr : a.ch), a.n_src, a.wgt, a.bias, a.cout, a.D, a.h, a.w, a.sz, a.sxy, a.relu, a.skip,
                                                    a.out, a.n_smp, (a.null_ss ? nullptr : a.ss), a.skip_ss, a.out_ss, nullptr)
                         : effi_conv3d_k3_f32(a.srcs, (a.null_ch ? nullptr : a.ch), a.n_src, a.wgt, a.bias, a.cout, a.D, a.h, a.w, a.sz, a.sxy, a.relu, a.skip, a.out,
                                              nullptr);
    emit(batch ? "effi_conv3d_k3_f32_batch" : "effi_conv3d_k3_f32", batch ? label + L(" n_smp%d", a.n_smp) : label, rc);
    return g_rec;
}
static ConvArgs conv_at(int cin, int cout, int sz, int sxy, int D = 6, int h = 37, int w = 50) {
// ... 979 lines not shown
```

effi_mvs_plus_amd/csrc/volume_ops.hip:

```cpp
#include <cstdint>
#include "common.hpp"
#include "launch_form.hpp"

namespace {

constexpr int TPB = 256;

__global__ __launch_bounds__(TPB) void planar_to_nhwc_kernel(EffiPtrList srcs, EffiOutList dsts, int C, int HW) {
    extern __shared__ __attribute__((aligned(16))) float tile[];
    const float* __restrict__ src = srcs.p[blockIdx.y];
    float* __restrict__ dst = dsts.p[blockIdx.y];
    const long p0 = (long)blockIdx.x * 64;
    const int n = C * 64;
    for (int e = threadIdx.x; e < n; e += TPB) {
        const int c = e >> 6, p = e & 63;
        const long gp = p0 + p;
        tile[c * 65 + p] = (gp < HW) ? src[(long)c * HW + gp] : 0.0f;
    }
    __syncthreads();
    for (int e = threadIdx.x; e < n; e += TPB) {
        const int p = e / C, c = e - p * C;
        const long gp = p0 + p;
        if (gp < HW) dst[gp * C + c] = tile[c * 65 + p];
    }
// ... 81 lines not shown
        const long t = i / W;
        const int y = (int)(t % H);
        const int c = (int)(t / H);
        out[i] = in[((long)c * h + y / f) * w + x / f];
    }
}

__global__ __launch_bounds__(TPB) void head_update_kernel(const float* __restrict__ s9, const float* __restrict__ bias2,
                                                          const float* __restrict__ inv, const float* __restrict__ disp_range,
                                                          int n_range, int h, int w, float* __restrict__ out_inv,
                                                          float* __restrict__ out_depth) {
    const int wq = w >> 2;
    const long q = (long)blockIdx.x * TPB + threadIdx.x;
    if (q >= (long)h * wq) return;
    const int y = (int)(q / wq), x = (int)(q - (long)y * wq) * 4;
    const long hw = (long)h * w;
    float acc[4] = {0.0f, 0.0f, 0.0f, 0.0f};
#pragma unroll
    for (int ky = 0; ky < 3; ++ky) {
        const int yy = y + ky - 1;
        if (yy < 0 || yy >= h) continue;
        const float* row = s9 + (long)yy * w + x;
#pragma unroll
        for (int kx = 0; kx < 3; ++kx) {
            const float* pl = row + (long)(ky * 3 + kx) * hw;
            const float4 c = *reinterpret_cast<const float4*>(pl);
            if (kx == 0) {
                const float l = (x > 0) ? pl[-1] : 0.0f;
                acc[0] = acc[0] + l; acc[1] = acc[1] + c.x; acc[2] = acc[2] + c.y; acc[3] = acc[3] + c.z;
            } else if (kx == 1) {
                acc[0] = acc[0] + c.x; acc[1] = acc[1] + c.y; acc[2] = acc[2] + c.z; acc[3] = acc[3] + c.w;
            } else {
                const float r = (x + 4 < w) ? pl[4] : 0.0f;
                acc[0] = acc[0] + c.y; acc[1] = acc[1] + c.z; acc[2] = acc[2] + c.w; acc[3] = acc[3] + r;
            }
        }
    }
    const float b = bias2[0], lo = disp_range[0], hi = disp_range[n_range - 1];
    const long pix = (long)y * w + x;
    const float4 iv = *reinterpret_cast<const float4*>(inv + pix);
    float4 o, d;
    o.x = iv.x + tanhf(acc[0] + b); o.y = iv.y + tanhf(acc[1] + b); o.z = iv.z + tanhf(acc[2] + b); o.w = iv.w + tanhf(acc[3] + b);
    d.x = effi_inv_to_depth(o.x, lo, hi); d.y = effi_inv_to_depth(o.y, lo, hi);
    d.z = effi_inv_to_depth(o.z, lo, hi); d.w = effi_inv_to_depth(o.w, lo, hi);
    *reinterpret_cast<float4*>(out_inv + pix) = o;
    *reinterpret_cast<float4*>(out_depth + pix) = d;
}

__device__ __forceinline__ void view_aggregate_body(const float* __restrict__ sim_views, const float* __restrict__ weights,
                                                    int S, int D, int hw, float* __restrict__ out) {
    const int p = blockIdx.x * TPB + threadIdx.x;
    if (p >= hw) return;
    const int d0 = blockIdx.y * 8;
    if (!weights) {
        for (int d = d0; d < min(D, d0 + 8); ++d) {
            float acc = 0.0f;
            for (int v = 0; v < S; ++v) acc = acc + sim_views[((long)v * D + d) * hw + p];
            out[(long)d * hw + p] = acc / (float)S;
        }
        return;
    }
    float wv[EFFI_MAX_VIEWS];
    float wsum = 0.0f;
#pragma unroll
    for (int v = 0; v < EFFI_MAX_VIEWS; ++v) {
        wv[v] = (v < S) ? weights[(long)v * hw + p] : 0.0f;
        if (v < S) wsum = wsum + wv[v];
    }
    const float den = wsum + 1e-6f;
    for (int d = d0; d < min(D, d0 + 8); ++d) {
        float acc = 0.0f;
#pragma unroll
        for (int v = 0; v < EFFI_MAX_VIEWS; ++v)
            if (v < S) acc = acc + sim_views[((long)v * D + d) * hw + p] * wv[v];
        out[(long)d * hw + p] = acc / den;
    }
}

__global__ void view_aggregate_kernel(const float* __restrict__ sim_views, const float* __restrict__ weights,
                                      int S, int D, int hw, float* __restrict__ out) {
    view_aggregate_body(sim_views, weights, S, D, hw, out);
}
__global__ void view_aggregate_batch_kernel(const float* __restrict__ sim_views, long sim_ss, const float* __restrict__ weights, long w_ss,
                                            int S, int D, int hw, float* __restrict__ out, long out_ss) {
    const long smp = blockIdx.z;
    view_aggregate_body(sim_views + smp * sim_ss, weights ? weights + smp * w_ss : nullptr, S, D, hw, out + smp * out_ss);
}

__device__ __forceinline__ void conf_store_up(float* __restrict__ out_up, float conf, int p, int w, int f) {
    const int y = p / w, x = p - y * w;
    float* dst = out_up + ((long)y * f) * ((long)w * f) + (long)x * f;
    if (f == 4) {
        const float4 v = make_float4(conf, conf, conf, conf);
#pragma unroll
        for (int j = 0; j < 4; ++j) *reinterpret_cast<float4*>(dst + (long)j * w * 4) = v;
        return;
    }
    for (int j = 0; j < f; ++j)
        for (int i = 0; i < f; ++i) dst[(long)j * w * f + i] = conf;
}

__device__ __forceinline__ void softmax_regress_conf_body(const float* __restrict__ logits, const float* __restrict__ depth,
                                                          long dds, long dps, int D, int hw,
                                                          float* __restrict__ out_depth, float* __restrict__ out_conf,
                                                          const float* __restrict__ disp_range, int n_range, float* __restrict__ out_dinv,
                                                          float* __restrict__ out_conf_up, int w, int f) {
    const int p = blockIdx.x * blockDim.x + threadIdx.x;
    if (p >= hw) return;
    float m = -INFINITY;
    for (int d = 0; d < D; ++d) m = fmaxf(m, logits[(long)d * hw + p]);
    float sum = 0.0f;
    for (int d = 0; d < D; ++d) sum = sum + expf(logits[(long)d * hw + p] - m);
    float dep = 0.0f, idxf = 0.0f;
    for (int d = 0; d < D; ++d) {
        const float pr = expf(logits[(long)d * hw + p] - m) / sum;
        dep = dep + pr * depth[d * dds + p * dps];
        idxf = idxf + pr * (float)d;
    }
    int idx = (int)idxf;
    idx = max(0, min(D - 1, idx));
    float s4 = 0.0f;
    for (int k = idx - 1; k <= idx + 2; ++k) {
        const float pr = (k >= 0 && k < D) ? expf(logits[(long)k * hw + p] - m) / sum : 0.0f;
        s4 = s4 + pr;
    }
    out_depth[p] = dep;
    const float conf = 4.0f * (s4 / 4.0f);
    out_conf[p] = conf;
// ... 35 lines not shown
#pragma unroll
    for (int d = 0; d < DT; ++d) dv[d] = depth[d * dds + p * dps];
    float m = -INFINITY;
#pragma unroll
    for (int d = 0; d < DT; ++d) m = fmaxf(m, e[d]);
    float sum = 0.0f;
#pragma unroll
    for (int d = 0; d < DT; ++d) {
        e[d] = expf(e[d] - m);
        sum = sum + e[d];
    }
    float dep = 0.0f, idxf = 0.0f;
#pragma unroll
    for (int d = 0; d < DT; ++d) {
        e[d] = e[d] / sum;
        dep = dep + e[d] * dv[d];
        idxf = idxf + e[d] * (float)d;
    }
    int idx = (int)idxf;
    idx = max(0, min(DT - 1, idx));
    float s4 = 0.0f;
#pragma unroll
    for (int d = 0; d < DT; ++d) {
        const bool in = (d >= idx - 1) & (d <= idx + 2);
        s4 = in ? s4 + e[d] : s4;
    }
    out_depth[p] = dep;
    const float conf = 4.0f * (s4 / 4.0f);
    out_conf[p] = conf;
    if (out_dinv) out_dinv[p] = effi_depth_to_inv(dep, disp_range[0], disp_range[n_range - 1]);
    if (out_conf_up) conf_store_up(out_conf_up, conf, p, w, f);
}

template <int DT>
__global__ __launch_bounds__(64) void softmax_regress_conf_reg_kernel(const float* __restrict__ logits, const float* __restrict__ depth,
                                                                      long dds, long dps, int hw, float* __restrict__ out_depth,
                                                                      float* __restrict__ out_conf, const float* __restrict__ disp_range,
                                                                      int n_range, float* __restrict__ out_dinv,
                                                                      float* __restrict__ out_conf_up, int w, int f) {
    softmax_regress_conf_reg_body<DT>(logits, depth, dds, dps, hw, out_depth, out_conf, disp_range, n_range, out_dinv, out_conf_up, w, f);
}
template <int DT>
__global__ __launch_bounds__(64) void softmax_regress_conf_reg_batch_kernel(const float* __restrict__ logits, const float* __restrict__ depth,
                                                                            long dds, long dps, int hw, float* __restrict__ out_depth,
                                                                            float* __restrict__ out_conf,
                                                                            const float* __restrict__ disp_range, int n_range,
                                                                            float* __restrict__ out_dinv, float* __restrict__ out_conf_up,
                                                                            int w, int f, SoftmaxBatch b) {
    const long s = blockIdx.y;
    softmax_regress_conf_reg_body<DT>(logits + s * b.logits, depth + s * b.depth, dds, dps, hw, out_depth + s * b.out_depth,
                                      out_conf + s * b.out_conf, disp_range ? disp_range + s * b.range : nullptr, n_range,
                                      out_dinv ? out_dinv + s * b.out_dinv : nullptr, out_conf_up ? out_conf_up + s * b.out_conf_up : nullptr,
                                      w, f);
}

__device__ __forceinline__ float lookup1d(const float* __restrict__ vol, long dstride, int Dp,
                                          float q_depth, float dmin, float dmax) {
    int x0;
    float w0, w1;
    lookup1d_index(Dp, q_depth, dmin, dmax, x0, w0, w1);
    return lookup1d_fetch(vol, dstride, Dp, x0, w0, w1);
}

__global__ void bilinear_sampler1d_kernel(const float* __restrict__ img, int C, int W, const float* __restrict__ coords, long nq,
                                          long total, float* __restrict__ out, float* __restrict__ mask) {
    const long i = (long)blockIdx.x * TPB + threadIdx.x;
    if (i >= total) return;
    const long n = i / nq, q = i - n * nq;
    const float xp = coords[2 * i], yp = coords[2 * i + 1];
    const float wm1 = (float)(W - 1);
    const float g = 2.0f * xp / wm1 - 1.0f;
    float ix = ((g + 1.0f) / 2.0f) * wm1;
    ix = fminf(fmaxf(ix, -2.0f), wm1 + 2.0f);
    const float x0f = floorf(ix);
    const int x0 = (int)x0f;
    const float w1 = ix - x0f, w0 = (x0f + 1.0f) - ix;
    const float* row = img + n * (long)C * W;
    for (int c = 0; c < C; ++c) out[(n * C + c) * nq + q] = lookup1d_fetch(row + (long)c * W, 1, W, x0, w0, w1);
    if (mask) mask[i] = ((g > -1.0f) & (yp > -1.0f) & (g < 1.0f) & (yp < 1.0f)) ? 1.0f : 0.0f;
}

__global__ void vol_lookup1d_kernel(const float* __restrict__ vol, long vds, long vps, int Dp,
                                    const float* __restrict__ query, long qds, long qys, long qxs, int nq,
                                    const float* __restrict__ dmin, const float* __restrict__ dmax, long rps,
                                    int h, int w, float* __restrict__ out, const float* __restrict__ vol_b,
                                    float* __restrict__ out_b) {
    const int p = blockIdx.x * TPB + threadIdx.x;
    if (p >= h * w) return;
    if (blockIdx.y) {
        vol = vol_b;
        out = out_b;
    }
    const int y = p / w, x = p - y * w;
    const float lo = dmin[p * rps], hi = dmax[p * rps];
    const float* v = vol + p * vps;
    for (int k = 0; k < nq; ++k) {
        const float q = query[k * qds + y * qys + x * qxs];
        out[(long)k * h * w + p] = lookup1d(v, vds, Dp, q, lo, hi);
    }
}

__global__ void getcost_kernel(const float* __restrict__ inv_depth, const float* __restrict__ disp_range,
                               int n_range, int input_is_depth, const float* __restrict__ interval,
                               const float* __restrict__ cur_vol, long cds, long cps, int Dcur,
                               const float* __restrict__ reg_vol, long rds, long rps_, int Dreg,
                               const float* __restrict__ dmin, const float* __restrict__ dmax, long range_ps,
                               int nq, int hw, float* __restrict__ cost) {
    const int p = blockIdx.x * TPB + threadIdx.x;
    if (p >= hw) return;
    const float itv = interval[0];
    float depth = inv_depth[p];
    if (!input_is_depth) depth = effi_inv_to_depth(depth, disp_range[0], disp_range[n_range - 1]);
    const float dv = 1.0f / depth;
    const float half = (float)(nq / 2) * itv;
// ... 632 lines not shown
```

effi_mvs_plus_amd/models/Effi_MVS_plus.py:

```python
from __future__ import annotations

from functools import partial

import torch
import torch.nn as nn

from .. import ops, packing
from .module import (ConvBnReLU, CostRegNet_2_sample_FPN3D_Fast, P_1to8_FeatureNet_Fast, _require_eval,
                     cost_up_small, mvs_loss)
from .update import BasicUpdateBlock

Align_Corners_Range = False


def _stack(ts):
    return ts[0].unsqueeze(0) if len(ts) == 1 else torch.stack(ts)


def disp_to_depth(disp, min_depth, max_depth):
    lo, hi = 1 / max_depth, 1 / min_depth
    scaled = (lo + (hi - lo) * disp).clamp(min=1e-4)
    return scaled, 1 / scaled


# ... 21 lines not shown


@ops.on_tensor_device
def upsample_depth(depth, mask, ratio=8):
    if ratio != 2:
        raise NotImplementedError("upsample_depth: the HIP path instantiates ratio 2 (feat_ratio of every stage)")
    return _stack([ops.convex_upsample2x(depth[n].contiguous(), mask[n].contiguous())[0] for n in range(depth.shape[0])])


class PixelwiseNet2d(nn.Sequential):

    def __init__(self):
        super().__init__(ConvBnReLU(1, 16), ConvBnReLU(16, 16), ConvBnReLU(16, 8), nn.Conv2d(8, 1, 1), nn.Sigmoid())
        self._cache = packing.PackCache()

    def run(self, entropy):
        _require_eval(self)
        t = []
        for i in range(3):
            t += [self[i].conv.weight, self[i].bn.weight, self[i].bn.bias, self[i].bn.running_mean, self[i].bn.running_var]
        t += [self[3].weight, self[3].bias]
        return ops.pixelwise_net(entropy, self._cache.get(t, lambda: packing.pack_pixelwise_net(self)))

    @ops.on_tensor_device
    def forward(self, x):
        n, c, h, w = x.shape
        return self.run(x.reshape(n * c, h, w).contiguous()).view(n, c, h, w)


def cascade_setup(disp_range, pairs, D1):
    if len(pairs) <= 4 and ops.option("setup_fused"):
        (hyp, misc), rts = ops.cascade_setup(disp_range, D1, pairs)
        return hyp, misc, rts
    rel = (lambda ps: ops.compose_rel_proj_stages(ps)) if len(pairs) <= 4 else (lambda ps: [ops.compose_rel_proj(p_) for p_ in ps])
    if disp_range.dim() == 1:
        return (*ops.stage1_hypotheses(disp_range, D1), rel(pairs))
    hm = [ops.stage1_hypotheses(r, D1) for r in disp_range]
    per = [rel([p_[b] for p_ in pairs]) for b in range(len(hm))]
    return (torch.stack([x[0] for x in hm]), torch.stack([x[1] for x in hm]),
            [torch.stack([r[s] for r in per]) for s in range(len(pairs))])


def stage1_volume(maps, rt, hyp, D, cost_regularization, pixel_wise_net, disp_range=None, x3=False):
    if isinstance(maps, ops.ViewTable):
        sim_views, entropy = ops.warpcorr_views_tbl(maps, 0, rt, hyp, D, x3=x3)
    else:
        sim_views, entropy = ops.warpcorr_views(maps[0], maps[1:], rt, hyp, D, x3=x3)
    if pixel_wise_net is None:
        weights = None
    elif hasattr(pixel_wise_net, "run"):
        weights = pixel_wise_net.run(entropy)
    else:
        weights = pixel_wise_net(entropy.reshape((-1, 1) + entropy.shape[-2:])).squeeze(1).contiguous().view(entropy.shape)
    cur_vol = ops.view_aggregate(sim_views, weights)
    reg_vol = cost_regularization.run(cur_vol.unsqueeze(-4))[0].select(-4, 0)
    inv_next = conf_up = None
    if disp_range is None:
        depth, conf = ops.softmax_regress_conf(reg_vol, hyp)
    elif ops.option("conf_fused"):
        depth, conf, inv_next, conf_up = ops.softmax_regress_conf(reg_vol, hyp, disp_range, conf_up=4)
    else:
        depth, conf, inv_next = ops.softmax_regress_conf(reg_vol, hyp, disp_range)
    return weights, cur_vol, reg_vol, depth, conf, inv_next, conf_up


class DepthNet(nn.Module):
    def __init__(self, cnnpixel=False):
        super().__init__()

    @staticmethod
    def run(feats, pairs, depth, num_depth, cost_regularization, pixel_wise_net):
        weights, volume, reg, d, conf, _, _ = stage1_volume(ops.to_nhwc(feats), ops.compose_rel_proj(pairs), depth, num_depth,
                                                            cost_regularization, pixel_wise_net)
        return {"depth": d, "photometric_confidence": conf, **({"view_weights": weights} if weights is not None else {}),
                "reg_volume": reg, "volume": volume.unsqueeze(-4)}

    @ops.on_tensor_device
    def forward(self, features, proj_matrices, depth_values, num_depth, cost_regularization, pixel_wise_net, G=8):
        assert len(features) == proj_matrices.shape[1], "Different number of images and projection matrices"
        assert depth_values.shape[1] == num_depth, "depth_values.shape[1]:{}  num_depth:{}".format(
            depth_values.shape[1], num_depth)
        if G != 1:
            raise NotImplementedError("DepthNet: group-wise correlation is instantiated for G=1 (the shipped model)")
        if self.training:
            if pixel_wise_net is None:
                raise NotImplementedError("DepthNet (training): the unweighted average (pixel_wise_net=None) has no backward on the "
                                          "HIP path; the shipped model always passes its PixelwiseNet")
            from .. import train_path
            return train_path.depthnet(pixel_wise_net, cost_regularization, features, proj_matrices, depth_values)
        if features[0].shape[0] > 1 and hasattr(cost_regularization, "run"):
            pairs = proj_matrices if proj_matrices[0].is_contiguous() else proj_matrices.contiguous()
            res = self.run(list(features), pairs, depth_values, num_depth, cost_regularization, pixel_wise_net)
            if pixel_wise_net is None:
                res["view_weights"] = []
            return res
        outs = []
        for b in range(features[0].shape[0]):
            outs.append(self.run([f[b] for f in features], proj_matrices[b].contiguous(), depth_values[b], num_depth,
                                 cost_regularization, pixel_wise_net))
        res = {k: _stack([o[k] for o in outs]) for k in outs[0]}
        if pixel_wise_net is None:
            res["view_weights"] = []
        return res


class GetCost_initvolume(nn.Module):
    def __init__(self):
        super().__init__()
# ... 182 lines not shown
                  and all(ctx[k].shape[-1] % 4 == 0 for k in keys))

        state_q4 = [False] * self.num_stage

        def all_states():
            nonlocal sr_maps, state_q4
            cs = [ctx[k].contiguous() for k in keys]
            if use_sr:
                nm = BasicUpdateBlock.N_SR_MAPS
                sr_maps = [ops.sr_alloc(nm, self.hdim_stage[s], cs[s].shape[1], cs[s].shape[2], cs[s].device, clear=False)
                           for s in range(self.num_stage)]
                clear_fused = bool(ops.option("clear_fused"))
                if not clear_fused:
                    ops.sr_clear_border(sr_maps)
                state_q4 = [self.update_block[s].state_q4_ok(not want_intermediates) and ops.uses_sr(cs[s].shape[1] * cs[s].shape[2])
                            for s in range(self.num_stage)]
                return dict(enumerate(ops.split_tanh_relu_stages_sr(cs, self.hdim_stage[:self.num_stage], self.cdim_stage[:self.num_stage],
                                                                    [m[-1] for m in sr_maps], q4=state_q4,
                                                                    clear=sr_maps if clear_fused else None)))
            if self.num_stage <= 4:
                return dict(enumerate(ops.split_tanh_relu_stages(cs, self.hdim_stage[:self.num_stage], self.cdim_stage[:self.num_stage])))
            return {s: ops.split_tanh_relu(cs[s], self.hdim_stage[s], self.cdim_stage[s]) for s in range(self.num_stage)}

        geo = {0: geometry(0) if stage1 is None else ((), rts[0], feats[0][keys[0]].shape)}
        with ops.Branch() as prep_branch:
            st = all_states()
            for s in range(1, self.num_stage):
                geo[s] = geometry(s)
        prep_joined = False
        tail_branch = None
        inv_next = None
        for s in range(self.num_stage):
            if s > 0:
                ops.mark("stage{}".format(s))
            nhwc, rt, (_, h, w) = geo[s]
            if s == 0:
                weights, cur_vol, reg_vol, depth, c, inv_next, conf = [stage1[k] for k in self._STAGE1_KEYS] if stage1 is not None else \
                    stage1_volume(table if table is not None else nhwc, rt, hyp, D1, self.cost_regularization, self.PixelwiseNet, disp_range,
                                  x3=bool(ops.option("warp_x3")))
                if conf is None:
                    with ops.Branch() as tail_branch:
                        conf = ops.upsample_nearest(c.unsqueeze(0), 4)[0]
                preds.append(depth)
                lo_cur, hi_cur = g_min, g_max
            else:
                D = self.depth_stage_nums[s]
                if table is not None:
                    sim, samples = ops.warpcorr_dyn_tbl(table, s, rt, preds[-1], misc[s:s + 1], weights, D)
                else:
                    sim, samples = ops.warpcorr_dyn(nhwc[0], nhwc[1:], rt, preds[-1], misc[s:s + 1], weights, D)
                x = sim.unsqueeze(0)
                csp_r, csp_c = self.CSP_R[s - 1], self.CSP_C[s - 1]
                if cur_vol.shape == reg_vol.shape and cur_vol.dim() == 3 and cost_up_small.pairable(csp_r, csp_c, x, w // 2):
                    prior, prior_c = ops.vol_lookup1d_pair(reg_vol, cur_vol, samples, lo_prev, hi_prev, h // 2, w // 2)
                    (reg_new, _), (cur_new, _) = cost_up_small.run_pair(csp_r, csp_c, x, prior.unsqueeze(0), prior_c.unsqueeze(0))
                    reg_vol, cur_vol = reg_new[0], cur_new[0]
                else:
                    with ops.Branch() as br:
                        prior_c = ops.vol_lookup1d(cur_vol, samples, lo_prev, hi_prev, h // 2, w // 2)
                        cur_new = csp_c.run(x, prior_c.unsqueeze(0))[0][0]
                    prior = ops.vol_lookup1d(reg_vol, samples, lo_prev, hi_prev, h // 2, w // 2)
                    reg_vol = csp_r.run(x, prior.unsqueeze(0))[0][0]
                    br.join(cur_new)
                    cur_vol = cur_new
                lo_cur, hi_cur = samples[D - 1], samples[0]
            if want_intermediates:
                inter["view_weights"] = weights
                inter["reg_volume{}".format(s + 1)] = reg_vol
                inter["cur_volume{}".format(s + 1)] = cur_vol
            if not prep_joined:
                prep_branch.join(*[t_ for k in st for t_ in st[k]], *[t_ for k in range(1, self.num_stage) for t_ in (list(geo[k][0]) + [geo[k][1]])])
                prep_joined = True
            hidden, inp = st[s]
            inv_cur = (inv_next if inv_next is not None else ops.depth_to_inv(preds[-1], disp_range)).unsqueeze(0)
            lookup = CostLookup(disp_range, misc[s:s + 1], cur_vol, reg_vol, lo_cur, hi_cur, self.CostNum)
            _, masks, invs, depths = self.update_block[s].run_fused(hidden, lookup, inv_cur, inp, self.seq_len[s],
                                                                     disp_range, fuse_upsample=not want_intermediates,
                                                                     sr_maps=None if sr_maps is None else sr_maps[s],
                                                                     net_sr_ready=sr_maps is not None, net_owned=True, net_q4=state_q4[s])
            preds.extend(d[0] for d in depths)
            if isinstance(masks[-1], tuple):
                up_depth, inv_next = masks[-1]
            else:
                _, up_depth, inv_next = ops.convex_upsample2x(invs[-1], masks[-1], disp_range, want_inv=False, want_depth_inv=True)
            preds.append(up_depth)
            lo_prev, hi_prev = lo_cur, hi_cur
        ops.mark("stage{}".format(self.num_stage))
        if tail_branch is not None:
            tail_branch.join(conf)
        out = {"depth": preds, "photometric_confidence": conf}
        if want_intermediates:
            out["intermediates"] = inter
        return out

    @ops.on_tensor_device
    def forward_hot(self, features, cnet_depth, proj_matrices, depth_values, want_intermediates=False):
        if self.training:
            from .. import train_path
            return train_path.hot_path(self, features, cnet_depth, proj_matrices, depth_values)
        B = depth_values.shape[0]
        if isinstance(features, ops.ViewTable) and B != 1:
            raise ValueError("forward_hot: a ViewTable describes ONE sample (B = 1)")
        stage1 = None
        if B > 1 and not isinstance(features, ops.ViewTable):
            stage1 = self._stage1_batch(features, proj_matrices, depth_values)
        outs = []
        for b in range(B):
            feats = features if isinstance(features, ops.ViewTable) else [{k: v[b] for k, v in f.items()} for f in features]
# ... 39 lines not shown
```

effi_mvs_plus_amd/models/module.py:

```python
from __future__ import annotations


import torch
import torch.nn as nn
import torch.nn.functional as F

from .. import ops, packing


def _require_eval(mod):
    if mod.training:
        raise NotImplementedError(
            f"{type(mod).__name__}.run is the fused inference launch; in training mode call the module itself (its forward takes "
            "the differentiable path of effi_mvs_plus_amd.train_path), or model.eval() for inference.")


def _stack(ts):
    return ts[0].unsqueeze(0) if len(ts) == 1 else torch.stack(ts)


def _triple(v):
    return tuple(v) if isinstance(v, (tuple, list)) else (v, v, v)


# ... 269 lines not shown
            (wu, bu), (wl, bl) = self._caches.setdefault("out3.split", packing.PackCache()).get(
                t, lambda: packing.pack_fpn_head_split(self.out3.weight, self.inner2.weight, self.inner2.bias))
            ones = self._ones.get((top.device, top.shape[-2], top.shape[-1]))
            if ones is None:
                ones = self._ones.setdefault((top.device, top.shape[-2], top.shape[-1]),
                                             torch.ones(1, top.shape[-2], top.shape[-1], device=top.device, dtype=torch.float32))
            u = ops.conv2d_k3_bf16x3([top, ones], wu, bu, 4 * co3)
            o3 = ops.conv2d_k3_bf16x3([l1], wl, bl, co3, epilogue=ops.EPI_NHWC_ADD_SHUF2 if cl else ops.EPI_ADD_SHUF2, aux0=u)
            out["stage3"] = o3.permute(*chw) if cl else o3
            return out
        w, b = self._pk("inner2", self.inner2)
        top = ops.conv2d([l1], w, b, self.inner2.out_channels, 1, epilogue=ops.EPI_ADD_UP2, aux0=top)
        out["stage3"] = head("out3", self.out3, top, 3)
        return out

    def forward_torch(self, x):
        l1 = self.conv1(self.conv0(x))
        l2 = self.conv2(l1)
        top = self.conv3(l2)
        outputs = {"stage1": self.out1(top)}
        top = F.interpolate(top, scale_factor=2, mode="nearest") + self.inner1(l2)
        outputs["stage2"] = self.out2(top)
        top = F.interpolate(top, scale_factor=2, mode="nearest") + self.inner2(l1)
        outputs["stage3"] = self.out3(top)
        return outputs

    @ops.on_tensor_device

    def forward(self, x):
        if self.training:
            from .. import train_path
            return train_path.feature_pyramid(self, x)
        if ops.option("fpn_batch") != 0 and x.shape[0] > 1:
            return self.run(x if x[0].is_contiguous() else x.contiguous())
        outs = [self.run(x[i].contiguous()) for i in range(x.shape[0])]
        return {k: _stack([o[k] for o in outs]) for k in outs[0]}


class CostRegNet_2_sample_FPN3D_Fast(nn.Module):
    def __init__(self, in_channels, base_channels):
        super().__init__()
        b = base_channels
        self.conv0 = Conv3d(in_channels, b, padding=1)
        self.conv1 = Conv3d(b, b, padding=1)
        self.conv2 = Conv3d(b, b * 2, stride=2, padding=1)
        self.conv3 = Conv3d(b * 2, b * 2, padding=1)
        self.conv4 = Conv3d(b * 2, b * 4, stride=2, padding=1)
        self.conv5 = Conv3d(b * 4, b * 4, padding=1)
        self.conv6 = Deconv3d(b * 4, b * 2, stride=2, padding=1, output_padding=1)
        self.conv7 = Deconv3d(b * 2, b, stride=2, padding=1, output_padding=1)
        self.prob = nn.Conv3d(b, 1, 3, stride=1, padding=1, bias=False)
        self._prob_cache = packing.PackCache()

    def run(self, vol):
        _require_eval(self)
        D, h, w = vol.shape[-3:]
        if D % 4 or h % 4 or w % 4:
            raise ValueError(f"cost volume dims {D}x{h}x{w} must be multiples of 4 (two stride-2 levels)")
        c1 = self.conv1.run([self.conv0.run([vol])])
        c3 = self.conv3.run([self.conv2.run([c1])])
        x = self.conv5.run([self.conv4.run([c3])])
        x = self.conv6.run(x, skip=c3)
        pro = self.conv7.run(x, skip=c1)
        wp, _ = self._prob_cache.get([self.prob.weight], lambda: packing.pack_conv3d(self.prob, None))
        prob = ops.conv3d_k3([pro], wp, None, 1, stride=(1, 1, 1), relu=False)
        return prob, pro

    @ops.on_tensor_device

    def forward(self, x):
        if self.training:
            from .. import train_path
            return train_path.cost_regnet(self, x)
        if x.shape[0] > 1:
            return self.run(x if x[0].is_contiguous() else x.contiguous())
        outs = [self.run(x[i].contiguous()) for i in range(x.shape[0])]
        return _stack([o[0] for o in outs]), _stack([o[1] for o in outs])


class cost_up_small(nn.Module):
    def __init__(self, in_channels, base_channels, IGEV_cost_channel=1):
        super().__init__()
        self.IGEV_cost_channel = IGEV_cost_channel
        self.conv0 = Conv3d(in_channels, base_channels, stride=(1, 2, 2), padding=1)
        self.conv_cost = Conv3d(self.IGEV_cost_channel, base_channels, padding=1)
        self.conv1 = Conv3d(base_channels * 2, base_channels, padding=1)
        self.conv2 = Deconv3d(base_channels, self.IGEV_cost_channel, stride=(1, 2, 2), padding=1,
                              output_padding=(0, 1, 1))

    def run(self, x, prior):
        a = self.conv0.run([x])
        b = self.conv_cost.run([prior])
        c1 = self.conv1.run([a, b])
        return self.conv2.run(c1), c1

    def _roll_packed(self):
        c = self.conv1
        t = [c.conv.weight, c.conv.bias] + ([c.bn.weight, c.bn.bias, c.bn.running_mean, c.bn.running_var] if c.bn is not None else [])
        return c._cache_roll.get(t, lambda: packing.pack_conv3d_roll_bf16x3(c.conv, c.bn))

    @staticmethod
    def pairable(a, b, x, prior_w):
        def stock(m):
            return (m.conv0.conv.in_channels == 1 and m.conv0.out_channels == 8 and _triple(m.conv0.conv.stride) == (1, 2, 2)
                    and m.conv_cost.conv.in_channels == 1 and m.conv_cost.out_channels == 8
                    and _triple(m.conv_cost.conv.stride) == (1, 1, 1) and m.conv1.out_channels == 8
                    and _triple(m.conv1.conv.stride) == (1, 1, 1) and m.conv2.out_channels == 1
                    and _triple(m.conv2.conv.stride) == (1, 2, 2) and m.conv0.relu and m.conv_cost.relu and m.conv1.relu
                    and m.conv2.relu and not m.training)
        if ops.option("csp_pair") == 0:
            return False
        return stock(a) and stock(b) and ops.uses_split() and x.shape[0] == 1 and prior_w % 4 == 0

    @staticmethod
    def run_pair(a, b, x, prior_a, prior_b):
        (w0a, b0a), (w0b, b0b) = a.conv0._packed(), b.conv0._packed()
        (wca, bca), (wcb, bcb) = a.conv_cost._packed(), b.conv_cost._packed()
        (w1a, b1a), (w1b, b1b) = a._roll_packed(), b._roll_packed()
        if ops.option("csp_gen") and x.shape[1] <= 14 and ops.get_option("roll_rp") != 0:
            c1a, c1b = ops.csp_gen_roll_pair(x, prior_a, w0a, b0a, wca, bca, w1a, b1a, prior_b, w0b, b0b, wcb, bcb, w1b, b1b)
        else:
            fa, fb = ops.conv3d_k3_pair(x, w0a, b0a, x, w0b, b0b, 8, sxy=2, relu=True)
            ga, gb = ops.conv3d_k3_pair(prior_a, wca, bca, prior_b, wcb, bcb, 8, sxy=1, relu=True)
            c1a, c1b = ops.conv3d_k3s1_roll_pair([fa, ga], w1a, b1a, [fb, gb], w1b, b1b, 8, relu=True)
        (w2a, b2a), (w2b, b2b) = a.conv2._packed(), b.conv2._packed()
        oa, ob = ops.deconv3d_k3_pair(c1a, w2a, b2a, c1b, w2b, b2b, 1, sz=1, relu=True)
        return (oa, c1a), (ob, c1b)

    @ops.on_tensor_device

    def forward(self, x, IGEV_cost):
        if self.training:
            from .. import train_path
            return train_path.cost_up_small(self, x, IGEV_cost)
        outs = [self.run(x[i].contiguous(), IGEV_cost[i].contiguous()) for i in range(x.shape[0])]
        return _stack([o[0] for o in outs]), _stack([o[1] for o in outs])


@ops.on_tensor_device
def homo_warping_new(src_fea, src_proj, ref_proj, depth_values):
    B, C_, H, W = src_fea.shape
    D = depth_values.shape[1]
    outs = []
    if src_fea.requires_grad and torch.is_grad_enabled():
        from .. import autograd as _ag
        for b in range(B):
            outs.append(_ag.homo_warp(src_fea[b], src_proj[b], ref_proj[b], depth_values[b]).reshape(C_, D * H, W))
        return torch.stack(outs)
    for b in range(B):
        nhwc = ops.to_nhwc([src_fea[b]])[0]
        rt = ops.rel_proj(src_proj[b].contiguous(), ref_proj[b].contiguous())
        dv = depth_values[b]
        outs.append(ops.homo_warp(nhwc, rt, dv if dv.dim() == 1 else dv, D).view(C_, D * H, W))
    return _stack(outs)


def depth_regression(p, depth_values):
    if depth_values.dim() <= 2:
        depth_values = depth_values.view(*depth_values.shape, 1, 1)
    return torch.sum(p * depth_values, 1)


def get_cur_depth_range_samples(cur_depth, ndepth, depth_inteval_pixel, shape, max_depth=192.0, min_depth=0.0):
    half = ndepth // 2 * depth_inteval_pixel
    lo = (cur_depth - half).clamp(min=1e-4)
    hi = (cur_depth + half).clamp(min=1e-4, max=1e4)
    assert cur_depth.shape == torch.Size(shape), "cur_depth:{}, input shape:{}".format(cur_depth.shape, shape)
    step = (hi - lo) / (ndepth - 1)
    idx = torch.arange(0, ndepth, device=cur_depth.device, dtype=cur_depth.dtype).reshape(1, -1, 1, 1)
    return (lo.unsqueeze(1) + idx * step.unsqueeze(1)).clamp(min=1e-5)


def get_depth_range_samples(cur_depth, ndepth, depth_inteval_pixel, device, dtype, shape, max_depth=192.0,
                            min_depth=0.0):
    if cur_depth.dim() == 2:
        lo, hi = cur_depth[:, 0], cur_depth[:, -1]
# ... 47 lines not shown
```

effi_mvs_plus_amd/ops.py:

```python
from __future__ import annotations

import collections
import ctypes as C
import functools
import os
import threading
from typing import NamedTuple

import weakref

import torch

from . import _lib
from ._lib import EffiLibraryError, check

ACT_NONE, ACT_RELU, ACT_SIGMOID, ACT_TANH = 0, 1, 2, 3
EPI_PLAIN, EPI_GRU_ZR, EPI_GRU_Q, EPI_HEAD, EPI_ADD_UP2, EPI_NHWC = 0, 1, 2, 3, 4, 5
EPI_ADD_SHUF2, EPI_NHWC_ADD_SHUF2 = 9, 10
MAX_VIEWS = 12


class KernelProfile:

    def __init__(self, keys=None):
# ... 5 lines not shown
        out, acc = {}, 0.0
        for key, _, e0, e1 in self.records:
            if e0 is None:
                out[key] = out.get(key, 0.0) + acc
                acc = 0.0
            else:
                acc += e0.elapsed_time(e1)
        return out

    def summary(self):
        torch.cuda.synchronize()
        out = {}
        for key, work, e0, e1 in self.records:
            if e0 is None:
                continue
            d = out.setdefault(key, {"launches": 0, "ms": 0.0, "flops": 0.0, "bytes": 0.0})
            d["launches"] += 1
            d["ms"] += e0.elapsed_time(e1)
            d["flops"] += work.get("flops", 0.0)
            d["bytes"] += work.get("bytes", 0.0)
        return out


_PROF = None

PRECISIONS = ("split", "fp32", "bf16")
_PRECISION = os.environ.get("EFFI_MVS_PRECISION", "split")
if _PRECISION not in PRECISIONS:
    raise ValueError(f"EFFI_MVS_PRECISION must be one of {PRECISIONS}, got {_PRECISION!r}")


def set_precision(mode):
    global _PRECISION
    if mode not in PRECISIONS:
        raise ValueError(f"precision must be one of {PRECISIONS}, got {mode!r}")
    _PRECISION = mode


def get_precision():
    return _PRECISION


def uses_split():
    return _PRECISION in ("split", "bf16")


def _x3(name):
    return getattr(_lib.lib(), name + "_bf16" if _PRECISION == "bf16" else name)


_PY_OPTION_DEFAULTS = {"warp_x3": 0, "state_q4": 1, "c1k7_mfma": 1, "k5s2_split": 1, "roll": 1, "conv3d_unaligned_split": 1, "conv3d_s2_split": 1, "fpn_conv0_fused": 1,
                       "fpn_split_head": 1, "csp_pair": 1, "head_taps": 1, "enc_tail": 0, "enc_gen": 1, "reduce_chunk": 2048, "gru_fused": 0, "csp_gen": 0,
                       "head_fused": 1, "head_fused_tile": 0, "clear_fused": 1, "setup_fused": 1, "conf_fused": 1,
                       "fpn_batch": 1}
_PY_OPTS = {k: int(os.environ.get("EFFI_" + k.upper(), v)) for k, v in _PY_OPTION_DEFAULTS.items()}
LIB_OPTIONS = ("warp_lds_kb", "dyn_form", "dyn_setup_exact", "dyn_xchg", "pixnet_mfma", "force_mr", "mr4_min", "mr4_nt2_max", "mr2_min",
               "wide_tiles", "roll_mr", "roll_zt", "roll_rp", "deconv_mr", "sr_waves", "enc_gen_mr3", "c3_lean", "dyn_win", "roll_slide")


def option(name):
    return _PY_OPTS[name]


def get_option(name):
    if name in _PY_OPTS:
        return _PY_OPTS[name]
    if name not in LIB_OPTIONS:
        raise KeyError(name)
    L = _lib.lib()
    v = L.effi_get_option(name.encode())
    return None if v == L.effi_option_unset() else int(v)


def set_option(name, value):
    before = get_option(name)
    if name in _PY_OPTS:
        _PY_OPTS[name] = _PY_OPTION_DEFAULTS[name] if value is None else int(value)
    else:
        L = _lib.lib()
        check(L.effi_set_option(name.encode(), L.effi_option_unset() if value is None else int(value)), "effi_set_option")
    return before


class options:

    def __init__(self, **kw):
        self.kw, self.before = kw, {}

    def __enter__(self):
        for k, v in self.kw.items():
            self.before[k] = set_option(k, v)
        return self

    def __exit__(self, *exc):
        for k, v in self.before.items():
            set_option(k, v)
        return False


LAUNCHERS = {"x3": 0, "x3_batch": 1, "x3_zb_batch": 2, "x3_pair": 3, "conv2d": 4, "planes3d": 5, "k5s2": 6, "s2_x3": 7, "roll": 8,
             "deconv_x3": 9, "c3_planes": 10, "deconv_k3": 11, "c3_zpt": 12}
LaunchForm = collections.namedtuple("LaunchForm", "rows cols waves planes variant")


def launch_form(launcher, h, w, nt=1, planes=1, count=1, cout=1, sr=False, zb=False, k1=False, s2=False, oct2=False):
    form = (C.c_int * 5)()
    flags = (1 if sr else 0) | (2 if zb else 0) | (4 if k1 else 0) | (8 if s2 else 0) | (16 if oct2 else 0)
    check(_lib.lib().effi_launch_form(LAUNCHERS[launcher], nt, h, w, planes, count, cout, flags, C.addressof(form)),
          "effi_launch_form")
    return LaunchForm(*form)
# ... 1458 lines not shown
        raise ValueError(mismatch)
    _, D, h, w = srcs_a[0].shape
    out_a = torch.empty(cout, *out_dims(D, h, w), device=srcs_a[0].device, dtype=torch.float32)
    return out_a, torch.empty_like(out_a), sum(s.shape[0] for s in srcs_a), D, h, w


def vol_lookup1d(vol, query, dmin, dmax, h, w):
    vol, vds, vps, Dp = _vol_strides(vol, h, w)
    nq, qds, qys, qxs = _query_strides(query, h, w)
    dmin_t, dmax_t, rps = _ranges(dmin, dmax, h, w)
    out = torch.empty(nq, h, w, device=query.device, dtype=torch.float32)
    check(_lib.lib().effi_vol_lookup1d_f32(_p(vol), vds, vps, Dp, _p(query), qds, qys, qxs, nq, _p(dmin_t),
                                            _p(dmax_t), rps, h, w, _p(out), _stream()), "effi_vol_lookup1d_f32")
    return out


def bilinear_sampler1d(img, coords, want_mask=False):
    _t(img, "img"), _t(coords, "coords")
    N, Cc, H, W = img.shape
    if H != 1 or coords.dim() != 4 or coords.shape[0] != N or coords.shape[-1] != 2:
        raise ValueError("bilinear_sampler1d: img [N,C,1,W] and coords [N,Ho,Wo,2]")
    Ho, Wo = coords.shape[1:3]
    out = torch.empty(N, Cc, Ho, Wo, device=img.device, dtype=torch.float32)
    mask = torch.empty(N, Ho, Wo, 1, device=img.device, dtype=torch.float32) if want_mask else None
    check(_lib.lib().effi_bilinear_sampler1d_f32(_p(img), N, Cc, W, _p(coords), Ho * Wo, _p(out), _p(mask), _stream()),
          "effi_bilinear_sampler1d_f32")
    return (out, mask) if want_mask else out


def vol_lookup1d_pair(vol_a, vol_b, query, dmin, dmax, h, w):
    vol_a, vds, vps, Dp = _vol_strides(vol_a, h, w)
    vol_b, vds_b, vps_b, Dp_b = _vol_strides(vol_b, h, w)
    if (vds, vps, Dp) != (vds_b, vps_b, Dp_b):
        raise ValueError("vol_lookup1d_pair: the two volumes must share shape and layout")
    nq, qds, qys, qxs = _query_strides(query, h, w)
    dmin_t, dmax_t, rps = _ranges(dmin, dmax, h, w)
    out_a = torch.empty(nq, h, w, device=query.device, dtype=torch.float32)
    out_b = torch.empty_like(out_a)
    check(_lib.lib().effi_vol_lookup1d_pair_f32(_p(vol_a), _p(vol_b), vds, vps, Dp, _p(query), qds, qys, qxs, nq, _p(dmin_t),
                                                 _p(dmax_t), rps, h, w, _p(out_a), _p(out_b), _stream()), "effi_vol_lookup1d_pair_f32")
    return out_a, out_b


def conv3d_k3_pair(x_a, weight_a, bias_a, x_b, weight_b, bias_b, cout, sxy=1, relu=True):
    out_a, out_b, cin, D, h, w = _pair_outputs([x_a], [x_b], "conv3d input", "conv3d_k3_pair: the two inputs must share their shape", cout,
                                               lambda D, h, w: (D, (h - 1) // sxy + 1, (w - 1) // sxy + 1))
    ho, wo = out_a.shape[2:]
    work = lambda: {"flops": 2.0 * 2 * 27 * cin * cout * D * ho * wo, "bytes": 2 * 4.0 * (cin * D * h * w + cout * D * ho * wo)}
    check(_call(f"conv3d_pair_c8_s1{sxy}", work, _lib.lib().effi_conv3d_k3_pair_f32, _p(x_a), _p(weight_a), _p(bias_a), _p(out_a),
                _p(x_b), _p(weight_b), _p(bias_b), _p(out_b), cin, cout, D, h, w, sxy, int(relu), _stream()), "effi_conv3d_k3_pair_f32")
    return out_a, out_b


def csp_gen_roll_pair(x, prior_a, w0_a, b0_a, wc_a, bc_a, w1_a, b1_a, prior_b, w0_b, b0_b, wc_b, bc_b, w1_b, b1_b):
    _t(x, "fine volume"), _t(prior_a, "prior"), _t(prior_b, "prior")
    _, D, H, W = x.shape
    h, w = (H - 1) // 2 + 1, (W - 1) // 2 + 1
    if tuple(prior_a.shape) != (1, D, h, w) or tuple(prior_b.shape) != (1, D, h, w):
        raise ValueError(f"csp_gen_roll_pair: priors must be [1,{D},{h},{w}], got {tuple(prior_a.shape)} / {tuple(prior_b.shape)}")
    for t_, n_ in ((w0_a, 216), (wc_a, 216), (w0_b, 216), (wc_b, 216), (b0_a, 8), (bc_a, 8), (b0_b, 8), (bc_b, 8)):
        _t(t_, "generated layer's parameters")
        if t_.numel() != n_:
            raise ValueError("csp_gen_roll_pair: the generated layers are 1 -> 8 channels (27 x 8 weights, 8 biases)")
    out_a = torch.empty(8, D, h, w, device=x.device, dtype=torch.float32)
    out_b = torch.empty_like(out_a)
    V = D * h * w
    work = lambda: {"flops": 2 * 2.0 * 27 * (8 * 2 + 16 * 8) * V, "bytes": 4.0 * (D * H * W + 2 * V + 2 * 8 * V)}
    check(_call("csp_gen_roll_pair", work, _x3("effi_csp_gen_roll_bf16x3_pair_f32"), _p(x), D, H, W, _p(prior_a), _p(w0_a), _p(b0_a),
                _p(wc_a), _p(bc_a), _p(w1_a), _p(b1_a), _p(out_a), _p(prior_b), _p(w0_b), _p(b0_b), _p(wc_b), _p(bc_b), _p(w1_b),
                _p(b1_b), _p(out_b), _stream()), "effi_csp_gen_roll_bf16x3_pair_f32")
    return out_a, out_b


def conv3d_k3s1_roll_pair(srcs_a, wpack_a, bias_a, srcs_b, wpack_b, bias_b, cout, relu=True):
    out_a, out_b, cin, D, h, w = _pair_outputs(srcs_a, srcs_b, "conv3d input",
                                               "conv3d_k3s1_roll_pair: the two source lists must share their shapes", cout)
    work = lambda: {"flops": 2 * 2.0 * 27 * cin * cout * D * h * w, "bytes": 2 * 4.0 * (cin + cout) * D * h * w}
    check(_call(f"conv3d_roll_pair_oct{cin // 8}", work, _x3("effi_conv3d_k3s1_roll_bf16x3_pair_f32"), _ptr_array(srcs_a),
                _p(wpack_a), _p(bias_a), _p(out_a), _ptr_array(srcs_b), _p(wpack_b), _p(bias_b), _p(out_b),
                _int_array([s.shape[0] for s in srcs_a]), len(srcs_a), cout, D, h, w, int(relu), _stream()),
          "effi_conv3d_k3s1_roll_bf16x3_pair_f32")
    return out_a, out_b


def deconv3d_k3_pair(x_a, weight_a, bias_a, x_b, weight_b, bias_b, cout, sz=1, relu=True):
    out_a, out_b, cin, D, h, w = _pair_outputs([x_a], [x_b], "deconv3d input", "deconv3d_k3_pair: the two inputs must share their shape", cout,
                                               lambda D, h, w: (sz * D, 2 * h, 2 * w))
    work = lambda: {"flops": 2 * 2.0 * 27 * cin * cout * D * h * w, "bytes": 2 * 4.0 * (cin * D * h * w + cout * sz * D * 4 * h * w)}
    check(_call("deconv3d_pair_c1_s1", work, _lib.lib().effi_deconv3d_k3_pair_f32, _p(x_a), _p(weight_a), _p(bias_a), _p(out_a),
                _p(x_b), _p(weight_b), _p(bias_b), _p(out_b), cin, cout, D, h, w, sz, int(relu), _stream()), "effi_deconv3d_k3_pair_f32")
    return out_a, out_b


def getcost(x, disp_range, interval, cur_vol, reg_vol, dmin, dmax, nq, h, w, input_is_depth=False, out=None):
    _t(x, "inv_depth"), _t(interval, "interval")
    look, _, _, _keep = _lookup_args(cur_vol, reg_vol, dmin, dmax, h, w)
    if out is None:
        out = torch.empty(2 * nq, h, w, device=x.device, dtype=torch.float32)
    n_range = 0 if disp_range is None else disp_range.numel()
    check(_lib.lib().effi_getcost_f32(_p(x), _p(disp_range), n_range, int(input_is_depth), _p(interval), *look, nq, h, w, _p(out), _stream()),
          "effi_getcost_f32")
    return out


def getcost_conv1x1(x, disp_range, interval, cur_vol, reg_vol, dmin, dmax, nq, h, w, weight, bias, cout, relu=True,
                    input_is_depth=False, out=None):
# ... 852 lines not shown
```

include/effi_mvs_hip.h:

```cpp
#ifndef EFFI_MVS_HIP_H
#define EFFI_MVS_HIP_H

#ifdef __cplusplus
extern "C" {
#endif

#define EFFI_OK               0
#define EFFI_ERR_BADARG      -1
#define EFFI_ERR_UNSUPPORTED -2
#define EFFI_ERR_LAUNCH      -3
#define EFFI_ERR_WORKSPACE   -4

#define EFFI_MAX_VIEWS 12
#define EFFI_MAX_SRC    3
#define EFFI_VIEW_TABLE_ROW (EFFI_MAX_VIEWS + 2)
#define EFFI_VIEW_TABLE_MAX 64

typedef void* effi_stream_t;

#define EFFI_ACT_NONE    0
#define EFFI_ACT_RELU    1
#define EFFI_ACT_SIGMOID 2
#define EFFI_ACT_TANH    3
#define EFFI_EPI_PLAIN   0
// ... 231 lines not shown
int effi_depth_to_inv_f32(const float* depth, const float* disp_range, int n_range, int n, float* inv,
                          effi_stream_t stream);
int effi_stage1_hypotheses_f32(const float* disp_range, int n_range, int D, float* depths,
                               float* intervals, effi_stream_t stream);
int effi_upsample_nearest_f32(const float* in, int C, int h, int w, int f, float* out, effi_stream_t stream);
int effi_head_update_f32(const float* partial9, const float* bias2, const float* inv_depth, const float* disp_range,
                         int n_range, int h, int w, float* out_inv, float* out_depth, effi_stream_t stream);

int effi_fusion_dynamic_filter_f32(const float* ref_depth, const float* src_depths, const float* ref_cam,
                                   const float* src_cams, int n_src, int h, int w, const float* ref_conf, int conf_h,
                                   int conf_w, float prob_threshold, int dh_view_num, float dist_base, float rel_diff_base,
                                   int relative, float* mats_scratch, float* out_depth, unsigned char* out_geo_mask,
                                   unsigned char* out_prob_mask, unsigned char* out_mask, float* out_points,
                                   float* out_reproj_xyd, effi_stream_t stream);

int effi_fusion_vis_filter_f32(const float* ref_depth, const float* reproj_xyd, int n, int n_src, int h, int w, float dist_base,
                               float rel_diff_base, int thres_view, int relative, unsigned char* masks, effi_stream_t stream);
int effi_fusion_points_f32(int mode, const float* in, long in_batch_stride, const float* depth, const float* cams, int n, int h,
                           int w, float* mats_scratch, float* out, effi_stream_t stream);

int effi_fusion_dtu_reproject_f32(const float* ref_depth, const float* src_depth, const float* ref_cam, const float* src_cam, int h,
                                  int w, int s, int e, float dist_base, float diff_base, float* mats_scratch, float* out5,
                                  unsigned char* masks, effi_stream_t stream);

int effi_warpcorr_views_x3_f32(const float* ref_nhwc, const float* const* src_nhwc, int S, const float* rt,
                               const float* depth, long depth_dstride, long depth_pstride,
                               int C, int h, int w, int D, float* sim_views, float* entropy, int hi_only,
                               effi_stream_t stream);
int effi_warpcorr_views_x3_tbl_f32(const float* const* view_table_dev, int S, const float* rt, const float* depth,
                                   long depth_dstride, long depth_pstride, int C, int h, int w, int D, float* sim_views,
                                   float* entropy, int hi_only, effi_stream_t stream);
int effi_warpcorr_views_bwd_f32(const float* ref_nhwc, const float* const* src_nhwc, int S, const float* rt,
                                const float* depth, long depth_dstride, long depth_pstride, int C, int h, int w, int D,
                                const float* grad_sim, float* grad_ref_nhwc, float* const* grad_src_nhwc,
                                effi_stream_t stream);
int effi_homo_warp_bwd_f32(const float* rt, const float* depth, long depth_dstride, long depth_pstride, int C, int h, int w,
                           int D, const float* grad_out, float* grad_src_nhwc, effi_stream_t stream);

int effi_vol_lookup1d_pair_f32(const float* vol_a, const float* vol_b, long vol_dstride, long vol_pstride, int Dp,
                               const float* query, long q_dstride, long q_ystride, long q_xstride, int nq, const float* dmin,
                               const float* dmax, long range_pstride, int h, int w, float* out_a, float* out_b,
                               effi_stream_t stream);
int effi_conv3d_k3_pair_f32(const float* in_a, const float* weight_a, const float* bias_a, float* out_a, const float* in_b,
                            const float* weight_b, const float* bias_b, float* out_b, int cin, int cout, int D, int h, int w,
                            int sxy, int relu, effi_stream_t stream);
int effi_conv3d_k3s1_roll_bf16x3_pair_f32(const float* const* srcs_a, const void* wpack_a, const float* bias_a, float* out_a,
                                          const float* const* srcs_b, const void* wpack_b, const float* bias_b, float* out_b,
                                          const int* src_channels, int n_src, int cout, int D, int h, int w, int relu,
                                          effi_stream_t stream);
int effi_csp_gen_roll_bf16x3_pair_f32(const float* x, int D, int H, int W, const float* prior_a, const float* w0_a, const float* b0_a,
                                      const float* wc_a, const float* bc_a, const void* w1_a, const float* b1_a, float* out_a,
                                      const float* prior_b, const float* w0_b, const float* b0_b, const float* wc_b, const float* bc_b,
                                      const void* w1_b, const float* b1_b, float* out_b, effi_stream_t stream);
int effi_debug_poison_lds(unsigned pattern, void* sink4, effi_stream_t stream);
int effi_debug_pk_war_probe(float* out, int blocks, int reps, int variant, effi_stream_t stream);
int effi_deconv3d_k3_pair_f32(const float* in_a, const float* weight_a, const float* bias_a, float* out_a, const float* in_b,
                              const float* weight_b, const float* bias_b, float* out_b, int cin, int cout, int D, int h, int w,
                              int sz, int relu, effi_stream_t stream);

int effi_image_prepare_u8_f32(const unsigned char* img_hwc, int src_h, int src_w, int channels, int dst_h, int dst_w,
                              float* out_chw, effi_stream_t stream);
int effi_resize_linear_f32(const float* in_chw, int channels, int src_h, int src_w, int dst_h, int dst_w, float* out_chw,
                           effi_stream_t stream);

int effi_images_prepare_batch_u8_f32(const unsigned char* imgs_vhwc, int n_views, int h, int w, float* out_vchw,
                                     effi_stream_t stream);
int effi_gt_pyramid_f32(const float* depth, const unsigned char* mask_u8, int thresh, const float* range, int n_smp, int h, int w,
                        float* const* depth_out, float* const* mask_out, effi_stream_t stream);


int effi_conv_wgrad_f32(const float* a, const float* b, int ca, int cb, int cb_total, int cb_off, int kd, int ks, int Da, int ha,
                        int wa, int Db, int hb, int wb, int sz, int sxy, float* dw, effi_stream_t stream);
int effi_conv2d_k5s2_dgrad_f32(const float* grad_out, const float* weight, int cin, int cout, int hin, int win, float* grad_in,
                               effi_stream_t stream);
int effi_channel_sum_f32(const float* g, int B, int C, long n, float* out, float* scratch, int nsplit, effi_stream_t stream);

int effi_bn_moment_f32(const float* x, int B, int C, long n, const float* shift, int power, float* out, float* scratch, int nsplit,
                       effi_stream_t stream);
int effi_bn_apply_f32(const float* x, int B, int C, long n, const float* mean, const float* invstd, const float* gamma,
                      const float* beta, int relu, float* y, effi_stream_t stream);
int effi_bn_train_fwd_f32(const float* x, int B, int C, long n, const float* gamma, const float* beta, float eps, float momentum,
                          float* running_mean, float* running_var, long long* n_tracked, int relu, float* y, float* mean,
                          float* invstd, float* scratch, int nsplit, effi_stream_t stream);
int effi_pack_conv2d_mfma_f32(const float* weight, const float* bias, int cout, int cin, int ks, int dgrad, float* wpack,
                              float* bias_pack, effi_stream_t stream);
int effi_pack_conv2d_k5s2_dgrad_f32(const float* weight, int cout, int cin, int ci_off, int ci_n, float* wpack, float* bias_pack,
                                    effi_stream_t stream);
int effi_bn_bwd_f32(const float* gy, const float* y, const float* x, int B, int C, long n, const float* mean, const float* invstd,
                    const float* gamma, int relu, float* s1, float* s2, float* gx, float* scratch, int nsplit,
                    effi_stream_t stream);

#define EFFI_PW_ACT_BWD_RELU     0
#define EFFI_PW_ACT_BWD_SIGMOID  1
#define EFFI_PW_ACT_BWD_TANH     2
#define EFFI_PW_TANH             3
#define EFFI_PW_RELU             4
#define EFFI_PW_SIGMOID          5
#define EFFI_PW_MUL              6
#define EFFI_PW_MUL_BWD          7
#define EFFI_PW_GRU              8
#define EFFI_PW_GRU_BWD          9
#define EFFI_PW_INV_TO_DEPTH     10
#define EFFI_PW_INV_TO_DEPTH_BWD 11
#define EFFI_PW_SCALE_CH         12
#define EFFI_PW_COUNT            13
int effi_pointwise_f32(int op, const float* a, const float* b, const float* c, const float* d, float s0, float s1, long n, long inner,
// ... 274 lines not shown
```

Baseline: 627.9 views/s.

## Fuse view aggregation and prior lookup into 1-to-8 channel 3-D conv tile loads

Adds producer-fused variants of the 1->8 channel 3x3x3 conv. One computes the weighted view aggregation of per-source similarity volumes directly into the LDS tile and writes the aggregated cost volume as a side output. Another performs the 1-D volume lookup of the prior while loading the tile. A third merges the stride-2 fine-volume conv pair and the lookup conv pair into a single launch (csp_entry4). The aim is to drop the intermediate aggregated and looked-up volumes and their separate kernel launches. The cost is redundant halo work: each tile recomputes the aggregation or lookup for its halo pixels across all views. A c3_planes option is also exposed for the plane-count picker.

```diff
diff --git a/effi_mvs_plus_amd/_lib.py b/effi_mvs_plus_amd/_lib.py
--- a/effi_mvs_plus_amd/_lib.py
+++ b/effi_mvs_plus_amd/_lib.py
@@ -86,6 +86,11 @@
     "effi_conv3d_k3_pair_f32": [_vp, _vp, _vp, _vp, _vp, _vp, _vp, _vp, _i, _i, _i, _i, _i, _i, _i, _vp],
     "effi_conv3d_k3s1_roll_bf16x3_pair_f32": [_vp, _vp, _vp, _vp, _vp, _vp, _vp, _vp, _vp, _i, _i, _i, _i, _i, _i, _vp],
     "effi_csp_gen_roll_bf16x3_pair_f32": [_vp, _i, _i, _i] + [_vp] * 16 + [_vp],
+    "effi_conv3d_c1to8_agg_f32": [_vp, _vp, _i, _i, _i, _i, _vp, _vp, _i, _vp, _vp, _vp],
+    "effi_conv3d_c1to8_lookup_pair_f32": [_vp, _vp, _l, _l, _i, _vp, _l, _l, _l, _vp, _vp, _l, _i, _i, _i, _vp, _vp, _vp, _vp, _vp, _vp, _i,
+                                          _vp],
+    "effi_csp_entry4_f32": [_vp, _i, _i, _i, _vp, _vp, _vp, _vp, _vp, _vp, _vp, _vp, _l, _l, _i, _vp, _l, _l, _l, _vp, _vp, _l, _vp, _vp,
+                            _vp, _vp, _vp, _vp, _i, _vp],
     "effi_debug_poison_lds": [C.c_uint, _vp, _vp],
     "effi_debug_pk_war_probe": [_vp, _i, _i, _i, _vp],
     "effi_deconv3d_k3_pair_f32": [_vp, _vp, _vp, _vp, _vp, _vp, _vp, _vp, _i, _i, _i, _i, _i, _i, _i, _vp],
diff --git a/effi_mvs_plus_amd/csrc/api.hip b/effi_mvs_plus_amd/csrc/api.hip
--- a/effi_mvs_plus_amd/csrc/api.hip
+++ b/effi_mvs_plus_amd/csrc/api.hip
@@ -42,7 +42,7 @@
 namespace {
 const char* const kOptName[EFFI_OPT_COUNT] = {"warp_lds_kb", "dyn_form", "dyn_setup_exact", "dyn_xchg", "pixnet_mfma", "force_mr", "mr4_min",
                                               "mr4_nt2_max", "mr2_min", "wide_tiles", "roll_mr", "roll_zt", "roll_rp", "deconv_mr", "sr_waves", "enc_gen_mr3", "c3_lean", "dyn_win",
-                                              "roll_slide"};
+                                              "roll_slide", "c3_planes"};
 long g_opt[EFFI_OPT_COUNT];
 std::once_flag g_opt_once;
 void load_options() {
@@ -99,7 +99,7 @@
         case EFFI_LF_S2_X3: f = effi_pick_s2_x3(h, w, nt == 1 ? 1 : (nt + 1) / 2, (long)planes * count); break;
         case EFFI_LF_ROLL: f = effi_pick_roll((flags & EFFI_LF_FLAG_OCT2) ? 2 : 1, nt, cout, h, w, planes, count, o); break;
         case EFFI_LF_DECONV_X3: f = effi_pick_deconv_x3(cout, h, w, planes, count, o); break;
-        case EFFI_LF_C3_PLANES: f = effi_pick_c3_planes(h, w, planes, count); break;
+        case EFFI_LF_C3_PLANES: f = effi_pick_c3_planes(h, w, planes, count, o); break;
         case EFFI_LF_DECONV_K3: f = effi_pick_deconv_k3(cout, h, w, planes, count); break;
         case EFFI_LF_C3_ZPT: f = EffiForm{1, EFFI_C3_TX, 4, effi_pick_c3_zpt(s2 ? 2 : 1, s2 ? 2 : 1, h, w, planes, nt, count), 0}; break;
         default: return EFFI_ERR_BADARG;
diff --git a/effi_mvs_plus_amd/csrc/common.hpp b/effi_mvs_plus_amd/csrc/common.hpp
--- a/effi_mvs_plus_amd/csrc/common.hpp
+++ b/effi_mvs_plus_amd/csrc/common.hpp
@@ -25,6 +25,7 @@
     EFFI_OPT_C3_LEAN,
     EFFI_OPT_DYN_WIN,
     EFFI_OPT_ROLL_SLIDE,
+    EFFI_OPT_C3_PLANES,
     EFFI_OPT_COUNT
 };
 constexpr long EFFI_OPT_UNSET = -0x7fffffffL;
@@ -185,6 +186,17 @@
     const float v0 = vol[lookup1d_tap0(Dp, x0) * dstride], v1 = vol[lookup1d_tap1(Dp, x0) * dstride];
     return lookup1d_blend(Dp, x0, w0, w1, v0, v1);
 }
+__device__ __forceinline__ float lookup1d(const float* __restrict__ vol, long dstride, int Dp, float q_depth, float dmin, float dmax) {
+    int x0;
+    float w0, w1;
+    lookup1d_index(Dp, q_depth, dmin, dmax, x0, w0, w1);
+    return lookup1d_fetch(vol, dstride, Dp, x0, w0, w1);
+}
+
+__device__ __forceinline__ float effi_view_den(float wsum) { return wsum + 1e-6f; }
+__device__ __forceinline__ float effi_view_term(float acc, float sim, float w, bool weighted) { return weighted ? acc + sim * w : acc + sim; }
+__device__ __forceinline__ float effi_view_finish(float acc, float den, int S, bool weighted) { return weighted ? acc / den : acc / (float)S; }
+
 __host__ __device__ inline bool effi_vol_fits32(long npix, long ps, int D, long ds) {
     return ps >= 0 && ds >= 0 && npix >= 1 && D >= 1 && ((npix - 1) * ps + (long)(D - 1) * ds + 1) * 4 < (1L << 31);
 }
diff --git a/effi_mvs_plus_amd/csrc/conv3d.hip b/effi_mvs_plus_amd/csrc/conv3d.hip
--- a/effi_mvs_plus_amd/csrc/conv3d.hip
+++ b/effi_mvs_plus_amd/csrc/conv3d.hip
@@ -197,13 +197,37 @@
     const float* bias;
     float* out;
 };
+enum { C1_PLAIN = 0, C1_AGG = 1, C1_LOOKUP = 2 };
+struct C1Agg {
+    const float* sim;
+    const float* weights;
+    int S;
+    float* cur;
+};
+struct C1Lookup {
+    const float* vol_a;
+    const float* vol_b;
+    long vds, vps;
+    int Dp;
+    const float* query;
+    long qds, qys, qxs;
+    const float* dmin;
+    const float* dmax;
+    long rps;
+};
 template <int SXY, int ZPT>
-__device__ __forceinline__ void conv3d_c1to8_body(const float* __restrict__ in, const float* __restrict__ wgt, const float* __restrict__ bias,
-                                                  float* __restrict__ out, int D, int h, int w, int ho, int wo, int relu) {
-    constexpr int IZ = ZPT + 2, IY = (TY - 1) * SXY + 3, IX = (TX - 1) * SXY + 3;
-    constexpr int PSZ = IY * IX, NPL = (PSZ + 255) / 256, PSZP = NPL * 256;
-    __shared__ float tile[IZ * PSZP];
-    __shared__ __attribute__((aligned(16))) float wl[27 * 8 + 8];
+struct C1Lds {
+    static constexpr int IZ = ZPT + 2, IY = (TY - 1) * SXY + 3, IX = (TX - 1) * SXY + 3;
+    static constexpr int PSZ = IY * IX, NPL = (PSZ + 255) / 256, PSZP = NPL * 256;
+    static constexpr int TILE = IZ * PSZP, WL = 27 * 8 + 8;
+};
+template <int SRC, int SXY, int ZPT, class Gen>
+__device__ __forceinline__ void conv3d_c1to8_body(float* __restrict__ tile, float* __restrict__ wl, const float* __restrict__ in, const Gen& gen,
+                                                  const float* __restrict__ wgt, const float* __restrict__ bias, float* __restrict__ out, int D,
+                                                  int h, int w, int ho, int wo, int relu) {
+    typedef C1Lds<SXY, ZPT> LD;
+    constexpr int IZ = LD::IZ, IX = LD::IX, PSZ = LD::PSZ, NPL = LD::NPL, PSZP = LD::PSZP;
+    static_assert(SRC == C1_PLAIN || SXY == 1, "the built sources are stride-1 layers");
 
     const int tid = threadIdx.x;
     const int tiles_x = (wo + TX - 1) / TX, tiles_xy = tiles_x * ((ho + TY - 1) / TY);
@@ -217,34 +241,123 @@
     if (tid < 27 * 8) wl[tid] = wgt[tid];
     if (tid < 8) wl[27 * 8 + tid] = bias ? bias[tid] : 0.0f;
 
-    int poff[NPL];
-#pragma unroll
-    for (int k = 0; k < NPL; ++k) {
-        const int e = tid + k * 256;
-        const int ly = e / IX, lx = e - ly * IX;
-        const int gy = iy0 + ly, gx = ix0 + lx;
-        poff[k] = ((e < PSZ) & (gy >= 0) & (gy < h) & (gx >= 0) & (gx < w)) ? gy * w + gx : -1;
-    }
-    float pf[IZ][NPL];
-    unsigned pb[NPL];
-#pragma unroll
-    for (int k = 0; k < NPL; ++k) pb[k] = (unsigned)max(poff[k], 0) * 4u;
-    const unsigned plane_b = (unsigned)(h * w) * 4u;
-#pragma unroll
-    for (int lz = 0; lz < IZ; ++lz) {
-        const int gz = iz0 + lz;
-        const bool zok = (gz >= 0) & (gz < D);
-        const unsigned so = (unsigned)min(max(gz, 0), D - 1) * plane_b;
+    if constexpr (SRC == C1_PLAIN) {
+        int poff[NPL];
 #pragma unroll
         for (int k = 0; k < NPL; ++k) {
-            const float t = *reinterpret_cast<const float*>(reinterpret_cast<const char*>(in) + (so + pb[k]));
-            pf[lz][k] = (zok & (poff[k] >= 0)) ? t : 0.0f;
-        }
-    }
-#pragma unroll
-    for (int lz = 0; lz < IZ; ++lz)
-#pragma unroll
-        for (int k = 0; k < NPL; ++k) tile[lz * PSZP + tid + k * 256] = pf[lz][k];
+            const int e = tid + k * 256;
+            const int ly = e / IX, lx = e - ly * IX;
+            const int gy = iy0 + ly, gx = ix0 + lx;
+            poff[k] = ((e < PSZ) & (gy >= 0) & (gy < h) & (gx >= 0) & (gx < w)) ? gy * w + gx : -1;
+        }
+        float pf[IZ][NPL];
+        unsigned pb[NPL];
+#pragma unroll
+        for (int k = 0; k < NPL; ++k) pb[k] = (unsigned)max(poff[k], 0) * 4u;
+        const unsigned plane_b = (unsigned)(h * w) * 4u;
+#pragma unroll
+        for (int lz = 0; lz < IZ; ++lz) {
+            const int gz = iz0 + lz;
+            const bool zok = (gz >= 0) & (gz < D);
+            const unsigned so = (unsigned)min(max(gz, 0), D - 1) * plane_b;
+#pragma unroll
+            for (int k = 0; k < NPL; ++k) {
+                const float t = *reinterpret_cast<const float*>(reinterpret_cast<const char*>(in) + (so + pb[k]));
+                pf[lz][k] = (zok & (poff[k] >= 0)) ? t : 0.0f;
+            }
+        }
+#pragma unroll
+        for (int lz = 0; lz < IZ; ++lz)
+#pragma unroll
+            for (int k = 0; k < NPL; ++k) tile[lz * PSZP + tid + k * 256] = pf[lz][k];
+    } else {
+        const unsigned hw = (unsigned)(h * w);
+        bool pok[NPL];
+        int cy[NPL], cx[NPL];
+#pragma unroll
+        for (int k = 0; k < NPL; ++k) {
+            const int e = tid + k * 256;
+            const int ly = e / IX, lx = e - ly * IX;
+            const int gy = iy0 + ly, gx = ix0 + lx;
+            pok[k] = (e < PSZ) & (gy >= 0) & (gy < h) & (gx >= 0) & (gx < w);
+            cy[k] = min(max(gy, 0), h - 1), cx[k] = min(max(gx, 0), w - 1);
+        }
+        unsigned cz[IZ];
+#pragma unroll
+        for (int lz = 0; lz < IZ; ++lz) cz[lz] = (unsigned)min(max(iz0 + lz, 0), D - 1);
+        if constexpr (SRC == C1_AGG) {
+            const bool weighted = gen.weights != nullptr;
+            unsigned pp[NPL];
+            float den[NPL], va[NPL][IZ];
+#pragma unroll
+            for (int k = 0; k < NPL; ++k) {
+                pp[k] = (unsigned)(cy[k] * w + cx[k]);
+                float wsum = 0.0f;
+                if (weighted)
+                    for (int v = 0; v < gen.S; ++v) wsum = wsum + gen.weights[v * hw + pp[k]];
+                den[k] = effi_view_den(wsum);
+#pragma unroll
+                for (int lz = 0; lz < IZ; ++lz) va[k][lz] = 0.0f;
+            }
+#pragma unroll 1
+            for (int v = 0; v < gen.S; ++v) {
+                const float* __restrict__ sv = gen.sim + (size_t)v * D * hw;
+                float sm[NPL][IZ], wk[NPL];
+#pragma unroll
+                for (int k = 0; k < NPL; ++k) {
+                    wk[k] = weighted ? gen.weights[v * hw + pp[k]] : 0.0f;
+#pragma unroll
+                    for (int lz = 0; lz < IZ; ++lz) sm[k][lz] = sv[cz[lz] * hw + pp[k]];
+                }
+#pragma unroll
+                for (int k = 0; k < NPL; ++k)
+#pragma unroll
+                    for (int lz = 0; lz < IZ; ++lz) va[k][lz] = effi_view_term(va[k][lz], sm[k][lz], wk[k], weighted);
+            }
+#pragma unroll
+            for (int k = 0; k < NPL; ++k)
+#pragma unroll
+                for (int lz = 0; lz < IZ; ++lz) {
+                    const int gz = iz0 + lz;
+                    va[k][lz] = effi_view_finish(va[k][lz], den[k], gen.S, weighted);
+                    tile[lz * PSZP + tid + k * 256] = ((gz >= 0) & (gz < D) & pok[k]) ? va[k][lz] : 0.0f;
+                }
+#pragma unroll
+            for (int k = 0; k < NPL; ++k) {
+                const int e = tid + k * 256;
+                const int ly = e / IX, lx = e - ly * IX;
+                const bool mine = pok[k] & (ly >= 1) & (ly <= TY) & (lx >= 1) & (lx <= TX);
+#pragma unroll
+                for (int lz = 1; lz <= ZPT; ++lz)
+                    if (mine && iz0 + lz < D) gen.cur[cz[lz] * hw + pp[k]] = va[k][lz];
+            }
+        } else {
+            const char* __restrict__ vb = reinterpret_cast<const char*>((blockIdx.y & 1) ? gen.vol_b : gen.vol_a);
+            const unsigned vds_b = (unsigned)gen.vds * 4u, qds = (unsigned)gen.qds;
+#pragma unroll
+            for (int k = 0; k < NPL; ++k) {
+                const unsigned p = (unsigned)(cy[k] * w + cx[k]);
+                const float lo = gen.dmin[p * (unsigned)gen.rps], hi = gen.dmax[p * (unsigned)gen.rps];
+                const unsigned pvb = p * (unsigned)gen.vps * 4u;
+                const float* __restrict__ qp = gen.query + ((unsigned)cy[k] * (unsigned)gen.qys + (unsigned)cx[k] * (unsigned)gen.qxs);
+                int x0[IZ];
+                float w0[IZ], w1[IZ], v0[IZ], v1[IZ];
+#pragma unroll
+                for (int lz = 0; lz < IZ; ++lz) lookup1d_index(gen.Dp, qp[cz[lz] * qds], lo, hi, x0[lz], w0[lz], w1[lz]);
+#pragma unroll
+                for (int lz = 0; lz < IZ; ++lz) {
+                    v0[lz] = *reinterpret_cast<const float*>(vb + (size_t)(pvb + (unsigned)lookup1d_tap0(gen.Dp, x0[lz]) * vds_b));
+                    v1[lz] = *reinterpret_cast<const float*>(vb + (size_t)(pvb + (unsigned)lookup1d_tap1(gen.Dp, x0[lz]) * vds_b));
+                }
+#pragma unroll
+                for (int lz = 0; lz < IZ; ++lz) {
+                    const int gz = iz0 + lz;
+                    const float t = lookup1d_blend(gen.Dp, x0[lz], w0[lz], w1[lz], v0[lz], v1[lz]);
+                    tile[lz * PSZP + tid + k * 256] = ((gz >= 0) & (gz < D) & pok[k]) ? t : 0.0f;
+                }
+            }
+        }
+    }
     __syncthreads();
 
     typedef float f2 __attribute__((ext_vector_type(2)));
@@ -293,18 +406,43 @@
         }
     }
 }
+struct C1None {};
 
 template <int SXY, int ZPT>
 __global__ __launch_bounds__(256) void conv3d_c1to8_kernel(C1Call ca, C1Call cb, int D, int h, int w, int ho, int wo, int relu) {
+    __shared__ float tile[C1Lds<SXY, ZPT>::TILE];
+    __shared__ __attribute__((aligned(16))) float wl[C1Lds<SXY, ZPT>::WL];
     const bool second = blockIdx.y != 0;
-    conv3d_c1to8_body<SXY, ZPT>(second ? cb.in : ca.in, second ? cb.wgt : ca.wgt, second ? cb.bias : ca.bias, second ? cb.out : ca.out, D, h,
-                                w, ho, wo, relu);
+    conv3d_c1to8_body<C1_PLAIN, SXY, ZPT>(tile, wl, second ? cb.in : ca.in, C1None{}, second ? cb.wgt : ca.wgt, second ? cb.bias : ca.bias,
+                                          second ? cb.out : ca.out, D, h, w, ho, wo, relu);
 }
 template <int SXY, int ZPT>
 __global__ __launch_bounds__(256) void conv3d_c1to8_batch_kernel(C1Call c, long in_ss, long out_ss, int D, int h, int w, int ho, int wo,
                                                                  int relu) {
+    __shared__ float tile[C1Lds<SXY, ZPT>::TILE];
+    __shared__ __attribute__((aligned(16))) float wl[C1Lds<SXY, ZPT>::WL];
     const long smp = blockIdx.y;
-    conv3d_c1to8_body<SXY, ZPT>(c.in + smp * in_ss, c.wgt, c.bias, c.out + smp * out_ss, D, h, w, ho, wo, relu);
+    conv3d_c1to8_body<C1_PLAIN, SXY, ZPT>(tile, wl, c.in + smp * in_ss, C1None{}, c.wgt, c.bias, c.out + smp * out_ss, D, h, w, ho, wo, relu);
+}
+template <int ZPT>
+__global__ __launch_bounds__(256) void conv3d_c1to8_agg_kernel(C1Agg g, C1Call c, int D, int h, int w, int relu) {
+    __shared__ float tile[C1Lds<1, ZPT>::TILE];
+    __shared__ __attribute__((aligned(16))) float wl[C1Lds<1, ZPT>::WL];
+    conv3d_c1to8_body<C1_AGG, 1, ZPT>(tile, wl, nullptr, g, c.wgt, c.bias, c.out, D, h, w, h, w, relu);
+}
+template <int ZPT, bool FOUR>
+__global__ __launch_bounds__(256) void conv3d_c1to8_entry_kernel(C1Call fa, C1Call fb, C1Lookup lk, C1Call ga, C1Call gb, int D, int H, int W,
+                                                                 int h, int w, int relu) {
+    __shared__ float tile[C1Lds<FOUR ? 2 : 1, ZPT>::TILE];
+    __shared__ __attribute__((aligned(16))) float wl[C1Lds<1, ZPT>::WL];
+    const bool second = (blockIdx.y & 1) != 0;
+    if (FOUR && blockIdx.y < 2) {
+        conv3d_c1to8_body<C1_PLAIN, 2, ZPT>(tile, wl, second ? fb.in : fa.in, C1None{}, second ? fb.wgt : fa.wgt, second ? fb.bias : fa.bias,
+                                            second ? fb.out : fa.out, D, H, W, h, w, relu);
+        return;
+    }
+    conv3d_c1to8_body<C1_LOOKUP, 1, ZPT>(tile, wl, nullptr, lk, second ? gb.wgt : ga.wgt, second ? gb.bias : ga.bias, second ? gb.out : ga.out,
+                                         D, h, w, h, w, relu);
 }
 
 static bool c3_lean(int bit) {
@@ -325,13 +463,27 @@
 int launch_c1to8(const C1Call& a, const C1Call* b, int D, int h, int w, int sxy, int relu, hipStream_t st, const C3Samples* bt = nullptr) {
     if (!effi_c1to8_fits32(D, h, w)) return EFFI_ERR_UNSUPPORTED;
     const int ho = (h - 1) / sxy + 1, wo = (w - 1) / sxy + 1, ncall = b ? 2 : bt ? bt->n : 1;
-    const int planes = effi_pick_c3_planes(ho, wo, D, ncall).planes;
+    const int planes = effi_pick_c3_planes(ho, wo, D, ncall, effi_form_opts()).planes;
     const dim3 grid(effi_cdiv(wo, TX) * effi_cdiv(ho, TY) * effi_cdiv(D, planes), ncall);
     return effi_switch<1, 2>(sxy, [&](auto SXY) {
         return effi_switch<4, 8>(planes, [&](auto ZPT) {
             if (bt) return effi_launch<conv3d_c1to8_batch_kernel<SXY(), ZPT()>>(grid, 256, st, a, bt->ss.src[0], bt->ss.out, D, h, w, ho, wo, relu);
             return effi_launch<conv3d_c1to8_kernel<SXY(), ZPT()>>(grid, 256, st, a, b ? *b : a, D, h, w, ho, wo, relu);
         });
+    });
+}
+int launch_c1to8_agg(const C1Agg& g, const C1Call& c, int D, int h, int w, int relu, hipStream_t st) {
+    const int planes = effi_pick_c3_planes(h, w, D, 1, effi_form_opts()).planes;
+    const dim3 grid(effi_cdiv(w, TX) * effi_cdiv(h, TY) * effi_cdiv(D, planes), 1);
+    return effi_switch<4, 8>(planes, [&](auto ZPT) { return effi_launch<conv3d_c1to8_agg_kernel<ZPT()>>(grid, 256, st, g, c, D, h, w, relu); });
+}
+int launch_c1to8_entry(const C1Call* fa, const C1Call* fb, const C1Lookup& lk, const C1Call& ga, const C1Call& gb, int D, int H, int W, int h,
+                       int w, int relu, hipStream_t st) {
+    const int ncall = fa ? 4 : 2, planes = effi_pick_c3_planes(h, w, D, ncall, effi_form_opts()).planes;
+    const dim3 grid(effi_cdiv(w, TX) * effi_cdiv(h, TY) * effi_cdiv(D, planes), ncall);
+    return effi_switch<4, 8>(planes, [&](auto ZPT) {
+        if (fa) return effi_launch<conv3d_c1to8_entry_kernel<ZPT(), true>>(grid, 256, st, *fa, *fb, lk, ga, gb, D, H, W, h, w, relu);
+        return effi_launch<conv3d_c1to8_entry_kernel<ZPT(), false>>(grid, 256, st, ga, gb, lk, ga, gb, D, h, w, h, w, relu);
     });
 }
 
@@ -524,7 +676,7 @@
 template <bool DECONV>
 int launch_c8to1(const C8Call& a, const C8Call* b, int D, int h, int w, int relu, hipStream_t st, const C3Samples* bt = nullptr) {
     if (!effi_c8to1_fits32(D, h, w)) return EFFI_ERR_UNSUPPORTED;
-    const int ncall = b ? 2 : bt ? bt->n : 1, planes = effi_pick_c3_planes(h, w, D, ncall).planes;
+    const int ncall = b ? 2 : bt ? bt->n : 1, planes = effi_pick_c3_planes(h, w, D, ncall, effi_form_opts()).planes;
     const dim3 grid(effi_cdiv(w, TX) * effi_cdiv(h, TY) * effi_cdiv(D, planes), ncall);
     return effi_switch<4, 8>(planes, [&](auto ZPT) {
         if (bt) return effi_launch<conv3d_c8to1_batch_kernel<DECONV, ZPT()>>(grid, 256, st, a, bt->ss.src[0], bt->ss.out, D, h, w, relu);
@@ -895,3 +1047,47 @@
     if (sz != 1 || cout != 1) return EFFI_ERR_UNSUPPORTED;
     return deconv3d_k3_run(a, &b, cin, cout, D, h, w, sz, relu, nullptr, stream);
 }
+
+extern "C" int effi_conv3d_c1to8_agg_f32(const float* sim_views, const float* weights, int S, int D, int h, int w, const float* weight,
+                                         const float* bias, int relu, float* cur_vol, float* out, effi_stream_t stream) {
+    if (!sim_views || !weight || !cur_vol || !out || S < 1 || S > EFFI_MAX_VIEWS || D < 1 || h < 1 || w < 1) return EFFI_ERR_BADARG;
+    if (!effi_c1to8_fits32(D, h, w)) return EFFI_ERR_UNSUPPORTED;
+    return launch_c1to8_agg(C1Agg{sim_views, weights, S, cur_vol}, C1Call{nullptr, weight, bias, out}, D, h, w, relu, effi_s(stream));
+}
+
+static int fill_c1_lookup(C1Lookup& lk, const float* vol_a, const float* vol_b, long vds, long vps, int Dp, const float* query, long qds,
+                          long qys, long qxs, const float* dmin, const float* dmax, long rps, int D, int h, int w) {
+    if (!vol_a || !vol_b || !query || !dmin || !dmax || Dp < 2 || D < 1 || h < 1 || w < 1) return EFFI_ERR_BADARG;
+    const long npix = (long)h * w;
+    if (!effi_c1to8_fits32(D, h, w) || !effi_vol_fits32(npix, vps, Dp, vds) || !effi_vol_fits32(npix, rps, 1, 0) || qds < 0 || qys < 0 ||
+        qxs < 0 || ((D - 1) * qds + (h - 1) * qys + (w - 1) * qxs + 1) * 4 >= (1L << 31))
+        return EFFI_ERR_UNSUPPORTED;
+    lk = C1Lookup{vol_a, vol_b, vds, vps, Dp, query, qds, qys, qxs, dmin, dmax, rps};
+    return EFFI_OK;
+}
+
+extern "C" int effi_conv3d_c1to8_lookup_pair_f32(const float* vol_a, const float* vol_b, long vds, long vps, int Dp, const float* query,
+                                                 long qds, long qys, long qxs, const float* dmin, const float* dmax, long rps, int D, int h,
+                                                 int w, const float* weight_a, const float* bias_a, float* out_a, const float* weight_b,
+                                                 const float* bias_b, float* out_b, int relu, effi_stream_t stream) {
+    C1Lookup lk;
+    if (!weight_a || !weight_b || !out_a || !out_b) return EFFI_ERR_BADARG;
+    if (const int rc = fill_c1_lookup(lk, vol_a, vol_b, vds, vps, Dp, query, qds, qys, qxs, dmin, dmax, rps, D, h, w)) return rc;
+    return launch_c1to8_entry(nullptr, nullptr, lk, C1Call{nullptr, weight_a, bias_a, out_a}, C1Call{nullptr, weight_b, bias_b, out_b}, D, h, w,
+                              h, w, relu, effi_s(stream));
+}
+
+extern "C" int effi_csp_entry4_f32(const float* x, int D, int H, int W, const float* w0_a, const float* b0_a, float* f_a, const float* w0_b,
+                                   const float* b0_b, float* f_b, const float* vol_a, const float* vol_b, long vds, long vps, int Dp,
+                                   const float* query, long qds, long qys, long qxs, const float* dmin, const float* dmax, long rps,
+                                   const float* wc_a, const float* bc_a, float* g_a, const float* wc_b, const float* bc_b, float* g_b, int relu,
+                                   effi_stream_t stream) {
+    C1Lookup lk;
+    if (!x || !w0_a || !w0_b || !f_a || !f_b || !wc_a || !wc_b || !g_a || !g_b || H < 1 || W < 1) return EFFI_ERR_BADARG;
+    const int h = (H - 1) / 2 + 1, w = (W - 1) / 2 + 1;
+    if (const int rc = fill_c1_lookup(lk, vol_a, vol_b, vds, vps, Dp, query, qds, qys, qxs, dmin, dmax, rps, D, h, w)) return rc;
+    if (!effi_c1to8_fits32(D, H, W)) return EFFI_ERR_UNSUPPORTED;
+    const C1Call fa{x, w0_a, b0_a, f_a}, fb{x, w0_b, b0_b, f_b};
+    return launch_c1to8_entry(&fa, &fb, lk, C1Call{nullptr, wc_a, bc_a, g_a}, C1Call{nullptr, wc_b, bc_b, g_b}, D, H, W, h, w, relu,
+                              effi_s(stream));
+}
diff --git a/effi_mvs_plus_amd/csrc/launch_form.hpp b/effi_mvs_plus_amd/csrc/launch_form.hpp
--- a/effi_mvs_plus_amd/csrc/launch_form.hpp
+++ b/effi_mvs_plus_amd/csrc/launch_form.hpp
@@ -34,6 +34,7 @@
     long wide_tiles;
     long sr_waves, roll_mr, roll_zt, roll_rp, deconv_mr;
     long roll_slide;
+    long c3_planes;
 };
 
 static inline long effi_opt_or(int id, long dflt) {
@@ -54,6 +55,7 @@
     o.roll_rp = effi_option(EFFI_OPT_ROLL_RP);
     o.deconv_mr = effi_option(EFFI_OPT_DECONV_MR);
     o.roll_slide = effi_opt_or(EFFI_OPT_ROLL_SLIDE, 1);
+    o.c3_planes = effi_option(EFFI_OPT_C3_PLANES);
     return o;
 }
 
@@ -154,9 +156,11 @@
     return EffiForm{mr2 ? 2 : 1, 16, 4, 1, 0};
 }
 
-static inline EffiForm effi_pick_c3_planes(int h, int w, int D, long ncall) {
+static inline EffiForm effi_pick_c3_planes(int h, int w, int D, long ncall, const EffiFormOpts& o) {
     const long tiles = (long)effi_cdiv(w, EFFI_C3_TX) * effi_cdiv(h, EFFI_C3_TY);
-    return EffiForm{1, EFFI_C3_TX, 4, tiles * effi_cdiv(D, 8) * ncall >= 512 ? 8 : 4, 0};
+    int planes = tiles * effi_cdiv(D, 8) * ncall >= 512 ? 8 : 4;
+    if (o.c3_planes != EFFI_OPT_UNSET) planes = (int)o.c3_planes;
+    return EffiForm{1, EFFI_C3_TX, 4, planes, 0};
 }
 
 static inline bool effi_c1to8_fits32(int D, int h, int w) { return (long)D * h * w < (1L << 29); }
diff --git a/effi_mvs_plus_amd/csrc/vol_host_check.cpp b/effi_mvs_plus_amd/csrc/vol_host_check.cpp
--- a/effi_mvs_plus_amd/csrc/vol_host_check.cpp
+++ b/effi_mvs_plus_amd/csrc/vol_host_check.cpp
@@ -16,6 +16,11 @@
 void show_one(const C3Batch& b) { FA(b, src, EFFI_MAX_SRC); FI(b, skip), FI(b, out); }
 void show_one(const Conv3dCall& c) { show_one(c.src); FP(c, wgt), FP(c, bias), FP(c, skip), FP(c, out); }
 void show_one(const C1Call& c) { FP(c, in), FP(c, wgt), FP(c, bias), FP(c, out); }
+void show_one(const C1Agg& g) { FP(g, sim), FP(g, weights), FI(g, S), FP(g, cur); }
+void show_one(const C1Lookup& l) {
+    FP(l, vol_a), FP(l, vol_b), FI(l, vds), FI(l, vps), FI(l, Dp), FP(l, query), FI(l, qds), FI(l, qys), FI(l, qxs), FP(l, dmin), FP(l, dmax),
+        FI(l, rps);
+}
 void show_one(const C8Call& c) { FP(c, in), FP(c, wgt), FP(c, bias), FP(c, out); }
 void show_one(const Deconv3dCall& c) { FP(c, in), FP(c, wgt), FP(c, bias), FP(c, skip), FP(c, out); }
 void show_one(const SoftmaxBatch& b) {
diff --git a/effi_mvs_plus_amd/csrc/volume_ops.hip b/effi_mvs_plus_amd/csrc/volume_ops.hip
--- a/effi_mvs_plus_amd/csrc/volume_ops.hip
+++ b/effi_mvs_plus_amd/csrc/volume_ops.hip
@@ -157,28 +157,27 @@
     const int p = blockIdx.x * TPB + threadIdx.x;
     if (p >= hw) return;
     const int d0 = blockIdx.y * 8;
-    if (!weights) {
-        for (int d = d0; d < min(D, d0 + 8); ++d) {
-            float acc = 0.0f;
-            for (int v = 0; v < S; ++v) acc = acc + sim_views[((long)v * D + d) * hw + p];
-            out[(long)d * hw + p] = acc / (float)S;
-        }
-        return;
-    }
+    const bool weighted = weights != nullptr;
     float wv[EFFI_MAX_VIEWS];
     float wsum = 0.0f;
-#pragma unroll
-    for (int v = 0; v < EFFI_MAX_VIEWS; ++v) {
-        wv[v] = (v < S) ? weights[(long)v * hw + p] : 0.0f;
-        if (v < S) wsum = wsum + wv[v];
-    }
-    const float den = wsum + 1e-6f;
+    if (weighted) {
+#pragma unroll
+        for (int v = 0; v < EFFI_MAX_VIEWS; ++v) {
+            wv[v] = (v < S) ? weights[(long)v * hw + p] : 0.0f;
+            if (v < S) wsum = wsum + wv[v];
+        }
+    }
+    const float den = effi_view_den(wsum);
     for (int d = d0; d < min(D, d0 + 8); ++d) {
         float acc = 0.0f;
-#pragma unroll
-        for (int v = 0; v < EFFI_MAX_VIEWS; ++v)
-            if (v < S) acc = acc + sim_views[((long)v * D + d) * hw + p] * wv[v];
-        out[(long)d * hw + p] = acc / den;
+        if (weighted) {
+#pragma unroll
+            for (int v = 0; v < EFFI_MAX_VIEWS; ++v)
+                if (v < S) acc = effi_view_term(acc, sim_views[((long)v * D + d) * hw + p], wv[v], true);
+        } else {
+            for (int v = 0; v < S; ++v) acc = effi_view_term(acc, sim_views[((long)v * D + d) * hw + p], 0.0f, false);
+        }
+        out[(long)d * hw + p] = effi_view_finish(acc, den, S, weighted);
     }
 }
 
@@ -320,14 +319,6 @@
                                       out_conf + s * b.out_conf, disp_range ? disp_range + s * b.range : nullptr, n_range,
                                       out_dinv ? out_dinv + s * b.out_dinv : nullptr, out_conf_up ? out_conf_up + s * b.out_conf_up : nullptr,
                                       w, f);
-}
-
-__device__ __forceinline__ float lookup1d(const float* __restrict__ vol, long dstride, int Dp,
-                                          float q_depth, float dmin, float dmax) {
-    int x0;
-    float w0, w1;
-    lookup1d_index(Dp, q_depth, dmin, dmax, x0, w0, w1);
-    return lookup1d_fetch(vol, dstride, Dp, x0, w0, w1);
 }
 
 __global__ void bilinear_sampler1d_kernel(const float* __restrict__ img, int C, int W, const float* __restrict__ coords, long nq,
diff --git a/effi_mvs_plus_amd/models/Effi_MVS_plus.py b/effi_mvs_plus_amd/models/Effi_MVS_plus.py
--- a/effi_mvs_plus_amd/models/Effi_MVS_plus.py
+++ b/effi_mvs_plus_amd/models/Effi_MVS_plus.py
@@ -97,8 +97,13 @@
         weights = pixel_wise_net.run(entropy)
     else:
         weights = pixel_wise_net(entropy.reshape((-1, 1) + entropy.shape[-2:])).squeeze(1).contiguous().view(entropy.shape)
-    cur_vol = ops.view_aggregate(sim_views, weights)
-    reg_vol = cost_regularization.run(cur_vol.unsqueeze(-4))[0].select(-4, 0)
+    if (ops.option("agg_fused") and sim_views.dim() == 4 and sim_views[0].numel() < 2 ** 29 and (weights is None or weights.is_contiguous())
+            and getattr(cost_regularization, "entry_fusable", lambda: False)()):
+        cur_vol, c0 = ops.conv3d_c1to8_agg(sim_views, weights, *cost_regularization.conv0._packed(), relu=True)
+        reg_vol = cost_regularization.run(cur_vol.unsqueeze(-4), c0=c0)[0].select(-4, 0)
+    else:
+        cur_vol = ops.view_aggregate(sim_views, weights)
+        reg_vol = cost_regularization.run(cur_vol.unsqueeze(-4))[0].select(-4, 0)
     inv_next = conf_up = None
     if disp_range is None:
         depth, conf = ops.softmax_regress_conf(reg_vol, hyp)
@@ -387,8 +392,12 @@
                 x = sim.unsqueeze(0)
                 csp_r, csp_c = self.CSP_R[s - 1], self.CSP_C[s - 1]
                 if cur_vol.shape == reg_vol.shape and cur_vol.dim() == 3 and cost_up_small.pairable(csp_r, csp_c, x, w // 2):
-                    prior, prior_c = ops.vol_lookup1d_pair(reg_vol, cur_vol, samples, lo_prev, hi_prev, h // 2, w // 2)
-                    (reg_new, _), (cur_new, _) = cost_up_small.run_pair(csp_r, csp_c, x, prior.unsqueeze(0), prior_c.unsqueeze(0))
+                    if cost_up_small.entry_fusable(x) and max(reg_vol.numel(), samples.numel()) < 2 ** 29:
+                        (reg_new, _), (cur_new, _) = cost_up_small.run_pair(csp_r, csp_c, x, None, None,
+                                                                            lookup=(reg_vol, cur_vol, samples, lo_prev, hi_prev))
+                    else:
+                        prior, prior_c = ops.vol_lookup1d_pair(reg_vol, cur_vol, samples, lo_prev, hi_prev, h // 2, w // 2)
+                        (reg_new, _), (cur_new, _) = cost_up_small.run_pair(csp_r, csp_c, x, prior.unsqueeze(0), prior_c.unsqueeze(0))
                     reg_vol, cur_vol = reg_new[0], cur_new[0]
                 else:
                     with ops.Branch() as br:
diff --git a/effi_mvs_plus_amd/models/module.py b/effi_mvs_plus_amd/models/module.py
--- a/effi_mvs_plus_amd/models/module.py
+++ b/effi_mvs_plus_amd/models/module.py
@@ -345,12 +345,18 @@
         self.prob = nn.Conv3d(b, 1, 3, stride=1, padding=1, bias=False)
         self._prob_cache = packing.PackCache()
 
-    def run(self, vol):
+    def entry_fusable(self):
+        c = self.conv0
+        return (not self.training and c.conv.in_channels == 1 and c.out_channels == 8 and _triple(c.conv.stride) == (1, 1, 1)
+                and _triple(c.conv.kernel_size) == (3, 3, 3) and _triple(c.conv.padding) == (1, 1, 1) and c.relu
+                and (ops.get_option("c3_lean") is None or ops.get_option("c3_lean") & 1))
+
+    def run(self, vol, c0=None):
         _require_eval(self)
         D, h, w = vol.shape[-3:]
         if D % 4 or h % 4 or w % 4:
             raise ValueError(f"cost volume dims {D}x{h}x{w} must be multiples of 4 (two stride-2 levels)")
-        c1 = self.conv1.run([self.conv0.run([vol])])
+        c1 = self.conv1.run([self.conv0.run([vol]) if c0 is None else c0])
         c3 = self.conv3.run([self.conv2.run([c1])])
         x = self.conv5.run([self.conv4.run([c3])])
         x = self.conv6.run(x, skip=c3)
@@ -406,15 +412,29 @@
         return stock(a) and stock(b) and ops.uses_split() and x.shape[0] == 1 and prior_w % 4 == 0
 
     @staticmethod
-    def run_pair(a, b, x, prior_a, prior_b):
+    def entry_fusable(x):
+        if not (ops.option("prior_fused") or ops.option("csp_entry4")):
+            return False
+        if ops.option("csp_gen") and x.shape[1] <= 14 and ops.get_option("roll_rp") != 0:
+            return False
+        return ops.get_option("c3_lean") is None or bool(ops.get_option("c3_lean") & 1)
+
+    @staticmethod
+    def run_pair(a, b, x, prior_a, prior_b, lookup=None):
         (w0a, b0a), (w0b, b0b) = a.conv0._packed(), b.conv0._packed()
         (wca, bca), (wcb, bcb) = a.conv_cost._packed(), b.conv_cost._packed()
         (w1a, b1a), (w1b, b1b) = a._roll_packed(), b._roll_packed()
         if ops.option("csp_gen") and x.shape[1] <= 14 and ops.get_option("roll_rp") != 0:
             c1a, c1b = ops.csp_gen_roll_pair(x, prior_a, w0a, b0a, wca, bca, w1a, b1a, prior_b, w0b, b0b, wcb, bcb, w1b, b1b)
         else:
-            fa, fb = ops.conv3d_k3_pair(x, w0a, b0a, x, w0b, b0b, 8, sxy=2, relu=True)
-            ga, gb = ops.conv3d_k3_pair(prior_a, wca, bca, prior_b, wcb, bcb, 8, sxy=1, relu=True)
+            if lookup is not None and ops.option("csp_entry4"):
+                fa, fb, ga, gb = ops.csp_entry4(x, w0a, b0a, w0b, b0b, *lookup, wca, bca, wcb, bcb, relu=True)
+            else:
+                fa, fb = ops.conv3d_k3_pair(x, w0a, b0a, x, w0b, b0b, 8, sxy=2, relu=True)
+                if lookup is not None:
+                    ga, gb = ops.conv3d_c1to8_lookup_pair(*lookup, fa.shape[2], fa.shape[3], wca, bca, wcb, bcb, relu=True)
+                else:
+                    ga, gb = ops.conv3d_k3_pair(prior_a, wca, bca, prior_b, wcb, bcb, 8, sxy=1, relu=True)
             c1a, c1b = ops.conv3d_k3s1_roll_pair([fa, ga], w1a, b1a, [fb, gb], w1b, b1b, 8, relu=True)
         (w2a, b2a), (w2b, b2b) = a.conv2._packed(), b.conv2._packed()
         oa, ob = ops.deconv3d_k3_pair(c1a, w2a, b2a, c1b, w2b, b2b, 1, sz=1, relu=True)
diff --git a/effi_mvs_plus_amd/ops.py b/effi_mvs_plus_amd/ops.py
--- a/effi_mvs_plus_amd/ops.py
+++ b/effi_mvs_plus_amd/ops.py
@@ -81,10 +81,11 @@
 _PY_OPTION_DEFAULTS = {"warp_x3": 0, "state_q4": 1, "c1k7_mfma": 1, "k5s2_split": 1, "roll": 1, "conv3d_unaligned_split": 1, "conv3d_s2_split": 1, "fpn_conv0_fused": 1,
                        "fpn_split_head": 1, "csp_pair": 1, "head_taps": 1, "enc_tail": 0, "enc_gen": 1, "reduce_chunk": 2048, "gru_fused": 0, "csp_gen": 0,
                        "head_fused": 1, "head_fused_tile": 0, "clear_fused": 1, "setup_fused": 1, "conf_fused": 1,
+                       "agg_fused": 1, "prior_fused": 0, "csp_entry4": 1,
                        "fpn_batch": 1}
 _PY_OPTS = {k: int(os.environ.get("EFFI_" + k.upper(), v)) for k, v in _PY_OPTION_DEFAULTS.items()}
 LIB_OPTIONS = ("warp_lds_kb", "dyn_form", "dyn_setup_exact", "dyn_xchg", "pixnet_mfma", "force_mr", "mr4_min", "mr4_nt2_max", "mr2_min",
-               "wide_tiles", "roll_mr", "roll_zt", "roll_rp", "deconv_mr", "sr_waves", "enc_gen_mr3", "c3_lean", "dyn_win", "roll_slide")
+               "wide_tiles", "roll_mr", "roll_zt", "roll_rp", "deconv_mr", "sr_waves", "enc_gen_mr3", "c3_lean", "dyn_win", "roll_slide", "c3_planes")
 
 
 def option(name):
@@ -1649,6 +1650,71 @@
     return out_a, out_b
 
 
+def _c1to8_params(*pairs):
+    for wt, b in pairs:
+        _t(wt, "1 -> 8 layer's weights")
+        if wt.numel() != 216 or (b is not None and _t(b, "1 -> 8 layer's bias").numel() != 8):
+            raise ValueError("a 1 -> 8 channel layer has 27 x 8 weights and 8 biases")
+
+
+def conv3d_c1to8_agg(sim_views, weights, weight, bias, relu=True, cur_out=None, out=None):
+    _t(sim_views, "sim_views")
+    S, D, h, w = sim_views.shape
+    if weights is not None and tuple(_t(weights, "weights").shape) != (S, h, w):
+        raise ValueError(f"conv3d_c1to8_agg: weights must be [{S},{h},{w}], got {tuple(weights.shape)}")
+    _c1to8_params((weight, bias))
+    cur = torch.empty(D, h, w, device=sim_views.device, dtype=torch.float32) if cur_out is None else _t(cur_out, "cur_out")
+    out = torch.empty(8, D, h, w, device=sim_views.device, dtype=torch.float32) if out is None else _t(out, "out")
+    if tuple(cur.shape) != (D, h, w) or tuple(out.shape) != (8, D, h, w):
+        raise ValueError("conv3d_c1to8_agg: cur_out must be [D,h,w] and out [8,D,h,w]")
+    V = D * h * w
+    work = lambda: {"flops": 2.0 * 27 * 8 * V + 2.0 * S * V, "bytes": 4.0 * (S * V + (S * h * w if weights is not None else 0) + 9 * V)}
+    check(_call("conv3d_c1to8_agg", work, _lib.lib().effi_conv3d_c1to8_agg_f32, _p(sim_views), _p(weights), S, D, h, w, _p(weight),
+                _p(bias), int(relu), _p(cur), _p(out), _stream()), "effi_conv3d_c1to8_agg_f32")
+    return cur, out
+
+
+def _prior_args(vol_a, vol_b, query, dmin, dmax, h, w, what):
+    vol_a, vds, vps, Dp = _vol_strides(vol_a, h, w)
+    vol_b, vds_b, vps_b, Dp_b = _vol_strides(vol_b, h, w)
+    if (vds, vps, Dp) != (vds_b, vps_b, Dp_b):
+        raise ValueError(what + ": the two volumes must share shape and layout")
+    nq, qds, qys, qxs = _query_strides(query, h, w)
+    dmin_t, dmax_t, rps = _ranges(dmin, dmax, h, w)
+    return (_p(vol_a), _p(vol_b), vds, vps, Dp, _p(query), qds, qys, qxs, _p(dmin_t), _p(dmax_t), rps), nq, (vol_a, vol_b, dmin_t, dmax_t)
+
+
+def conv3d_c1to8_lookup_pair(vol_a, vol_b, query, dmin, dmax, h, w, weight_a, bias_a, weight_b, bias_b, relu=True, outs=None):
+    args, D, keep = _prior_args(vol_a, vol_b, query, dmin, dmax, h, w, "conv3d_c1to8_lookup_pair")
+    _c1to8_params((weight_a, bias_a), (weight_b, bias_b))
+    out_a, out_b = outs if outs is not None else (torch.empty(8, D, h, w, device=query.device, dtype=torch.float32) for _ in range(2))
+    V = D * h * w
+    work = lambda: {"flops": 2 * 2.0 * 27 * 8 * V, "bytes": 2 * 4.0 * (2 * V + 8 * V)}
+    check(_call("conv3d_c1to8_lookup_pair", work, _lib.lib().effi_conv3d_c1to8_lookup_pair_f32, *args, D, h, w, _p(weight_a), _p(bias_a),
+                _p(_t(out_a, "out_a")), _p(weight_b), _p(bias_b), _p(_t(out_b, "out_b")), int(relu), _stream()),
+          "effi_conv3d_c1to8_lookup_pair_f32")
+    del keep
+    return out_a, out_b
+
+
+def csp_entry4(x, w0_a, b0_a, w0_b, b0_b, vol_a, vol_b, query, dmin, dmax, wc_a, bc_a, wc_b, bc_b, relu=True, outs=None):
+    _t(x, "fine volume")
+    _, D, H, W = x.shape
+    h, w = (H - 1) // 2 + 1, (W - 1) // 2 + 1
+    args, nq, keep = _prior_args(vol_a, vol_b, query, dmin, dmax, h, w, "csp_entry4")
+    if x.shape[0] != 1 or nq != D:
+        raise ValueError(f"csp_entry4: x must be [1,D,H,W] with one query plane per plane of x, got {tuple(x.shape)} and {nq} queries")
+    _c1to8_params((w0_a, b0_a), (w0_b, b0_b), (wc_a, bc_a), (wc_b, bc_b))
+    f_a, f_b, g_a, g_b = outs if outs is not None else (torch.empty(8, D, h, w, device=x.device, dtype=torch.float32) for _ in range(4))
+    V = D * h * w
+    work = lambda: {"flops": 4 * 2.0 * 27 * 8 * V, "bytes": 4.0 * (2 * D * H * W + 4 * V + 4 * 8 * V)}
+    check(_call("csp_entry4", work, _lib.lib().effi_csp_entry4_f32, _p(x), D, H, W, _p(w0_a), _p(b0_a), _p(_t(f_a, "f_a")), _p(w0_b), _p(b0_b),
+                _p(_t(f_b, "f_b")), *args, _p(wc_a), _p(bc_a), _p(_t(g_a, "g_a")), _p(wc_b), _p(bc_b), _p(_t(g_b, "g_b")), int(relu),
+                _stream()), "effi_csp_entry4_f32")
+    del keep
+    return f_a, f_b, g_a, g_b
+
+
 def csp_gen_roll_pair(x, prior_a, w0_a, b0_a, wc_a, bc_a, w1_a, b1_a, prior_b, w0_b, b0_b, wc_b, bc_b, w1_b, b1_b):
     _t(x, "fine volume"), _t(prior_a, "prior"), _t(prior_b, "prior")
     _, D, H, W = x.shape
diff --git a/include/effi_mvs_hip.h b/include/effi_mvs_hip.h
--- a/include/effi_mvs_hip.h
+++ b/include/effi_mvs_hip.h
@@ -307,6 +307,18 @@
                                       const float* wc_a, const float* bc_a, const void* w1_a, const float* b1_a, float* out_a,
                                       const float* prior_b, const float* w0_b, const float* b0_b, const float* wc_b, const float* bc_b,
                                       const void* w1_b, const float* b1_b, float* out_b, effi_stream_t stream);
+int effi_conv3d_c1to8_agg_f32(const float* sim_views, const float* weights, int S, int D, int h, int w, const float* weight,
+                              const float* bias, int relu, float* cur_vol, float* out, effi_stream_t stream);
+int effi_conv3d_c1to8_lookup_pair_f32(const float* vol_a, const float* vol_b, long vol_dstride, long vol_pstride, int Dp,
+                                      const float* query, long q_dstride, long q_ystride, long q_xstride, const float* dmin,
+                                      const float* dmax, long range_pstride, int D, int h, int w, const float* weight_a,
+                                      const float* bias_a, float* out_a, const float* weight_b, const float* bias_b, float* out_b,
+                                      int relu, effi_stream_t stream);
+int effi_csp_entry4_f32(const float* x, int D, int H, int W, const float* w0_a, const float* b0_a, float* f_a, const float* w0_b,
+                        const float* b0_b, float* f_b, const float* vol_a, const float* vol_b, long vol_dstride, long vol_pstride, int Dp,
+                        const float* query, long q_dstride, long q_ystride, long q_xstride, const float* dmin, const float* dmax,
+                        long range_pstride, const float* wc_a, const float* bc_a, float* g_a, const float* wc_b, const float* bc_b,
+                        float* g_b, int relu, effi_stream_t stream);
 int effi_debug_poison_lds(unsigned pattern, void* sink4, effi_stream_t stream);
 int effi_debug_pk_war_probe(float* out, int blocks, int reps, int variant, effi_stream_t stream);
 int effi_deconv3d_k3_pair_f32(const float* in_a, const float* weight_a, const float* bias_a, float* out_a, const float* in_b,
```

After: 631.9 views/s (median of 6 runs). About the same (+0.6%).
